# snap-research/GiGL

Measured on AMD Instinct MI355X. Metric: sampled+aggregated edges/s, higher is better.
Workload: dtype f32

## Files before the change

### gigl_amd/csrc/agg.hip

```cpp
#include "wave_reduce.h"
#include "common.h"

#include <cstring>

#include <cstdlib>
#include <type_traits>

#include <hip/hip_fp16.h>

__host__ __device__ static inline float hs_pow2_scale(float m) {
  uint32_t bits;
  memcpy(&bits, &m, 4);
  int e = (int)((bits >> 23) & 0xFF) - 127;
  if (((bits >> 23) & 0xFF) == 0) e = -126;
  int se = 14 - e;
  se = se > 60 ? 60 : (se < -60 ? -60 : se);
  const uint32_t sb = (uint32_t)(se + 127) << 23;
  float s;
  memcpy(&s, &sb, 4);
  return s;
}

namespace {

// ... 1090 lines not shown
        const _Float16 a1 = (_Float16)x;
        fa[s][0][e] = a1;
        fa[s][1][e] = (_Float16)(x - (float)a1);
      }
    if (c + 1 < nc) aload(c + 1);
    if (c + 1 == nc) w2load(0, nc & 1);
    if (c + 1 == nc && wv == 0) {
      short* dst = s_buf[nc & 1] + F2_IMG2;
      if (bias) __builtin_amdgcn_global_load_lds((gptr_t)(reinterpret_cast<const float4_t*>(bias) + lane), (lptr_t)dst, 16, 0, 0);
      else reinterpret_cast<float4_t*>(dst)[lane] = zero4;
    }
    const short* sw = s_buf[c & 1];
#pragma unroll
    for (int s = 0; s < 2; ++s) {
      if (c * 32 + 16 * s >= K) break;
#pragma unroll
      for (int tn = 0; tn < 2; ++tn) {
        half8v_t fw[4][2];
#pragma unroll
        for (int j = 0; j < 4; ++j)
#pragma unroll
          for (int p = 0; p < 2; ++p)
            fw[j][p] = *reinterpret_cast<const half8v_t*>(
                &sw[tn * F2_IMG1 + p * (F2_IMG1 / 2) + split_lds_off(j * 32 + r, 16 * s + 8 * g)]);
        constexpr int HA[3] = {1, 0, 0}, HW[3] = {0, 1, 0};
#pragma unroll
        for (int t = 0; t < 3; ++t)
#pragma unroll
          for (int j = 0; j < 4; ++j)
            acc[4 * tn + j] = __builtin_amdgcn_mfma_f32_32x32x16_f16(fw[j][HW[t]], fa[s][HA[t]], acc[4 * tn + j], 0, 0, 0);
      }
    }
    __syncthreads();
  }
  const float4_t* s_bias = reinterpret_cast<const float4_t*>(s_buf[nc & 1] + F2_IMG2);
  const float s_h = f2_scale[0], o2 = f2_scale[2];
  float16_t acc2[3];
#pragma unroll
  for (int n = 0; n < 3; ++n)
#pragma unroll
    for (int v = 0; v < 16; ++v) acc2[n][v] = 0.f;
#pragma unroll
  for (int rd = 0; rd < 8; ++rd) {
    const _Float16* sw2 = reinterpret_cast<const _Float16*>(s_buf[(nc + rd) & 1]);
    if (rd + 1 < 8) w2load(rd + 1, (nc + rd + 1) & 1);
#pragma unroll
    for (int hf = 0; hf < 2; ++hf) {
      half8v_t h1, h2;
#pragma unroll
      for (int q = 0; q < 2; ++q) {
        const float4_t bq = s_bias[8 * rd + 2 * (2 * hf + q) + g];
#pragma unroll
        for (int t = 0; t < 4; ++t) {
          float x = acc[rd][8 * hf + 4 * q + t] * hs_o + bq[t];
          x = (x > 0.f ? x : 0.f) * s_h;
          const _Float16 a1 = (_Float16)x;
          h1[4 * q + t] = a1;
          h2[4 * q + t] = (_Float16)(x - (float)a1);
        }
      }
#pragma unroll
      for (int n = 0; n < 3; ++n) {
        if (n == 2 && !wr_block) continue;
        const half8v_t w1 = *reinterpret_cast<const half8v_t*>(sw2 + split_lds_off(n * 32 + r, 16 * hf + 8 * g));
        const half8v_t w2 = *reinterpret_cast<const half8v_t*>(sw2 + F2_IMG2 / 2 + split_lds_off(n * 32 + r, 16 * hf + 8 * g));
        acc2[n] = __builtin_amdgcn_mfma_f32_32x32x16_f16(h2, w1, acc2[n], 0, 0, 0);
        acc2[n] = __builtin_amdgcn_mfma_f32_32x32x16_f16(h1, w2, acc2[n], 0, 0, 0);
        acc2[n] = __builtin_amdgcn_mfma_f32_32x32x16_f16(h1, w1, acc2[n], 0, 0, 0);
      }
    }
    if (rd + 1 < 8) __syncthreads();
  }
#pragma unroll
  for (int n = 0; n < 3; ++n) {
    if (n == 2 && !wr_block) continue;
#pragma unroll
    for (int v = 0; v < 16; ++v) {
      const int orow = m0b + wv * 32 + 8 * (v >> 2) + 4 * g + (v & 3);
      if (orow < M) y2[(int64_t)orow * F2_N2 + n * 32 + r] = acc2[n][v] * o2;
    }
  }
}

__global__ __launch_bounds__(256) void fused2_images_kernel(const float* __restrict__ hs, const float* __restrict__ f2,
                                                            const float* __restrict__ w1, int K, const float* __restrict__ w2,
                                                            int n_out, _Float16* __restrict__ w1img,
                                                            _Float16* __restrict__ w2img) {
  const int nc = (K + 31) >> 5;
  const int n1 = 2 * nc * 128 * 32, n2 = 2 * 4 * F2_N2 * 32;
  const int i = blockIdx.x * 256 + threadIdx.x;
  if (i < n1) {
    const int kpos = i & 31, c = (i >> 5) & 127, blk = i >> 12;
    const int tn = blk / nc, ch = blk - tn * nc;
    const int k = 32 * ch + f2_perm(kpos);
    const float x = k < K ? w1[(int64_t)(128 * tn + c) * K + k] * hs[1] : 0.f;
    const _Float16 a1 = (_Float16)x;
    _Float16* img = w1img + (int64_t)blk * F2_IMG1 + split_lds_off(c, kpos);
    img[0] = a1;
    img[F2_IMG1 / 2] = (_Float16)(x - (float)a1);
  } else if (i < n1 + n2) {
    const int e = i - n1;
    const int kpos = e & 31, rest = e >> 5, n = rest % F2_N2, blk = rest / F2_N2;
    const int k = 32 * blk + f2_perm(kpos);
    float x = 0.f;
    if (n < n_out) x = w2[(int64_t)n * 2 * F2_HID + k];
    else if (n >= F2_N2 / 2 && n - F2_N2 / 2 < n_out) x = w2[(int64_t)(n - F2_N2 / 2) * 2 * F2_HID + F2_HID + k];
    x *= f2[1];
    const _Float16 a1 = (_Float16)x;
    _Float16* img = w2img + (int64_t)blk * F2_IMG2 + split_lds_off(n, kpos);
    img[0] = a1;
    img[F2_IMG2 / 2] = (_Float16)(x - (float)a1);
  }
}

__global__ __launch_bounds__(256) void fused2_scale_kernel(const float* __restrict__ hs, const float* __restrict__ b1,
                                                           const float* __restrict__ w2, int n_w2, int K1,
                                                           float* __restrict__ f2) {
  __shared__ float s_m[2][4];
  const int tid = threadIdx.x, gt = blockIdx.x * 256 + tid, stride = gridDim.x * 256;
  float mb = 0.f, mw = 0.f;
  if (b1)
    for (int i = gt; i < F2_HID; i += stride) {
      const float v = fabsf(b1[i]);
      mb = fmaxf(mb, v == v ? v : 0.f);
    }
  for (int i = gt; i < n_w2; i += stride) {
    const float v = fabsf(w2[i]);
    mw = fmaxf(mw, v == v ? v : 0.f);
  }
#pragma unroll
  for (int o = 32; o >= 1; o >>= 1) {
    mb = fmaxf(mb, __shfl_xor(mb, o, 64));
    mw = fmaxf(mw, __shfl_xor(mw, o, 64));
  }
  if ((tid & 63) == 0) {
    s_m[0][tid >> 6] = mb;
    s_m[1][tid >> 6] = mw;
  }
  __syncthreads();
  if (tid == 0) {
    for (int i = 1; i < 4; ++i) {
      mb = fmaxf(mb, s_m[0][i]);
      mw = fmaxf(mw, s_m[1][i]);
    }
    uint32_t* acc = reinterpret_cast<uint32_t*>(f2) + 4;
    atomicMax(acc, __float_as_uint(mb));
    atomicMax(acc + 1, __float_as_uint(mw));
    __threadfence();
    if (atomicAdd(acc + 2, 1u) == gridDim.x - 1) {
      const float b = __uint_as_float(atomicExch(acc, 0u)), w = __uint_as_float(atomicExch(acc + 1, 0u));
      acc[2] = 0u;
      const float inf = __uint_as_float(0x7F800000u);
      float bound = (float)K1 * 1073741824.f * (1.f / hs[0]) * (1.f / hs[1]) + b;
      if (!(bound > 0.f) || !(bound < inf)) bound = 1.f;
      const float s_h = hs_pow2_scale(bound) * 0.5f;
      const float s_w2 = (w > 0.f && w < inf) ? hs_pow2_scale(w) : 1.f;
      f2[0] = s_h;
      f2[1] = s_w2;
      f2[2] = (1.f / s_h) * (1.f / s_w2);
    }
  }
}

__global__ __launch_bounds__(256) void hs_chain_kernel(const float* __restrict__ hs_prev, const float* __restrict__ b_prev,
                                                       int n_b, int k_prev, float fan, const float* __restrict__ w,
                                                       int64_t n_w, float* __restrict__ hs_out) {
  __shared__ float s_m[2][4];
  const int tid = threadIdx.x;
  const int64_t gt = (int64_t)blockIdx.x * 256 + tid, stride = (int64_t)gridDim.x * 256;
  float mb = 0.f, mw = 0.f;
  if (b_prev)
    for (int64_t i = gt; i < n_b; i += stride) {
      const float v = fabsf(b_prev[i]);
      mb = fmaxf(mb, v == v ? v : 0.f);
    }
  const float4* w4 = reinterpret_cast<const float4*>(w);
  const int64_t n4 = ((reinterpret_cast<uintptr_t>(w) & 15) == 0) ? n_w / 4 : 0;
  for (int64_t i = gt; i < n4; i += stride) {
    const float4 v = w4[i];
    const float a = fmaxf(fmaxf(fabsf(v.x), fabsf(v.y)), fmaxf(fabsf(v.z), fabsf(v.w)));
    mw = fmaxf(mw, a == a ? a : 0.f);
  }
  for (int64_t i = n4 * 4 + gt; i < n_w; i += stride) {
    const float v = fabsf(w[i]);
    mw = fmaxf(mw, v == v ? v : 0.f);
  }
#pragma unroll
  for (int o = 32; o >= 1; o >>= 1) {
    mb = fmaxf(mb, __shfl_xor(mb, o, 64));
    mw = fmaxf(mw, __shfl_xor(mw, o, 64));
  }
  if ((tid & 63) == 0) {
    s_m[0][tid >> 6] = mb;
    s_m[1][tid >> 6] = mw;
  }
  __syncthreads();
  if (tid == 0) {
    for (int i = 1; i < 4; ++i) {
      mb = fmaxf(mb, s_m[0][i]);
      mw = fmaxf(mw, s_m[1][i]);
    }
    uint32_t* acc = reinterpret_cast<uint32_t*>(hs_out) + 4;
    atomicMax(acc, __float_as_uint(mb));
    atomicMax(acc + 1, __float_as_uint(mw));
    __threadfence();
    if (atomicAdd(acc + 2, 1u) == gridDim.x - 1) {
      const float b = __uint_as_float(atomicExch(acc, 0u)), wm = __uint_as_float(atomicExch(acc + 1, 0u));
      acc[2] = 0u;
      const float inf = __uint_as_float(0x7F800000u);
      float bound = ((float)k_prev * 1073741824.f * (1.f / hs_prev[0]) * (1.f / hs_prev[1]) + b) * fan;
      if (!(bound > 0.f) || !(bound < inf)) bound = 1.f;
      const float s_h = hs_pow2_scale(bound) * 0.5f;
      const float s_w = (wm > 0.f && wm < inf) ? hs_pow2_scale(wm) : 1.f;
      hs_out[0] = s_h;
      hs_out[1] = s_w;
      hs_out[2] = (1.f / s_h) * (1.f / s_w);
    }
  }
}

template <int OP>
__global__ __launch_bounds__(256) void sage_fused_out_kernel(const float* __restrict__ p, const int32_t* __restrict__ rowptr,
                                                             const int32_t* __restrict__ rowend,
                                                             const int32_t* __restrict__ col,
                                                             const int32_t* __restrict__ root_local, int b, int n_out,
                                                             const float* __restrict__ bias, int act,
                                                             const int32_t* __restrict__ meta, float* __restrict__ out) {
  const int lane = threadIdx.x & 63, sub = lane >> 4, sl = lane & 15;
  const int s = (int)(((int64_t)blockIdx.x * blockDim.x + threadIdx.x) >> 6);
  if (s >= b) return;
  const bool failed = meta[GIGL_META_OVERFLOW] != 0;
  const int i = failed ? -1 : root_local[s];
  float* o = out + (int64_t)s * n_out;
  if (i < 0) {
    const float v = failed ? __builtin_nanf("") : 0.f;
    for (int c = lane; c < n_out; c += 64) o[c] = v;
    return;
  }
  const int e0 = rowptr[i], m = rowend[i] - e0;
  float4_t acc = {0.f, 0.f, 0.f, 0.f};
  if (sl < 12) {
    for (int e = sub; e < m; e += 8) {
// ... 2882 lines not shown

static int32_t linear_tiled_strided(gigl_ctx* ctx, const float* a_tiled, const float* w, const float* bias,
                                    const int32_t* m_dev, int64_t m_cap, int32_t k, int32_t n, int32_t act, float* y,
                                    int32_t ldy, int32_t batch = 1, int64_t a_bstride = 0, int64_t w_bstride = 0,
                                    const float* self_src = nullptr, const uint32_t* self_ids = nullptr,
                                    int32_t d_mean = 0, int32_t self_ld = 0, const float* hs_scale = nullptr, bool self_half = false) {
  const bool hs = hs_scale != nullptr;
  GIGL_REQUIRE(ctx, a_tiled && w && m_dev && y && (k & 3) == 0 && n > 0 && ldy >= n * batch && batch >= 1,
               "bad arguments");
  GIGL_HIP_CHECK(ctx, hipSetDevice(ctx->device));
  if (m_cap == 0) return GIGL_OK;
  hipStream_t st = ctx->stream;
  gigl_prof_scope ps(ctx, GIGL_K_LINEAR);
  const int nkc = (k + 31) / 32;
  const int64_t bm = (m_cap + 127) / 128;
  if (self_src) {
    GIGL_REQUIRE(ctx, batch == 1 && d_mean > 0 && (d_mean & 3) == 0 && d_mean < k && self_ld >= k - d_mean, "bad two-source operand");
    const int nkc_mean = (d_mean + 31) / 32;
    GIGL_REQUIRE(ctx, !self_half || hs, "fp16 self rows go with the half split");
    if (hs && self_half) {
      if (n > 64)
        hipLaunchKernelGGL((linear_split_kernel<2, true, true, false, true, true, true>), dim3((unsigned)(bm * ((n + 127) / 128)), 1u),
                           dim3(256), 0, st, a_tiled, w, bias, m_dev, k, n, act, y, nkc_mean, ldy, (int64_t)0, (int64_t)0,
                           self_src, self_ids, d_mean, self_ld, hs_scale);
      else
        hipLaunchKernelGGL((linear_split_kernel<1, true, true, false, true, true, true>), dim3((unsigned)(bm * ((n + 63) / 64)), 1u),
                           dim3(256), 0, st, a_tiled, w, bias, m_dev, k, n, act, y, nkc_mean, ldy, (int64_t)0, (int64_t)0,
                           self_src, self_ids, d_mean, self_ld, hs_scale);
      GIGL_HIP_CHECK(ctx, hipGetLastError());
      return GIGL_OK;
    }
    if (hs) {
      if (n > 64)
        hipLaunchKernelGGL((linear_split_kernel<2, true, true, false, true, true>), dim3((unsigned)(bm * ((n + 127) / 128)), 1u),
                           dim3(256), 0, st, a_tiled, w, bias, m_dev, k, n, act, y, nkc_mean, ldy, (int64_t)0, (int64_t)0,
                           self_src, self_ids, d_mean, self_ld, hs_scale);
      else
        hipLaunchKernelGGL((linear_split_kernel<1, true, true, false, true, true>), dim3((unsigned)(bm * ((n + 63) / 64)), 1u),
                           dim3(256), 0, st, a_tiled, w, bias, m_dev, k, n, act, y, nkc_mean, ldy, (int64_t)0, (int64_t)0,
                           self_src, self_ids, d_mean, self_ld, hs_scale);
      GIGL_HIP_CHECK(ctx, hipGetLastError());
      return GIGL_OK;
    }
    if (n > 64)
      hipLaunchKernelGGL((linear_split_kernel<2, true, true>), dim3((unsigned)(bm * ((n + 127) / 128)), 1u), dim3(256), 0, st,
                         a_tiled, w, bias, m_dev, k, n, act, y, nkc_mean, ldy, (int64_t)0, (int64_t)0, self_src, self_ids,
                         d_mean, self_ld);
    else
      hipLaunchKernelGGL((linear_split_kernel<1, true, true, false, false, true>), dim3((unsigned)(bm * ((n + 63) / 64)), 1u), dim3(256), 0, st,
                         a_tiled, w, bias, m_dev, k, n, act, y, nkc_mean, ldy, (int64_t)0, (int64_t)0, self_src, self_ids,
                         d_mean, self_ld);
    GIGL_HIP_CHECK(ctx, hipGetLastError());
    return GIGL_OK;
  }
  if (hs) {
    if (n > 64)
      hipLaunchKernelGGL((linear_split_kernel<2, true, false, false, true, true>), dim3((unsigned)(bm * ((n + 127) / 128)), (unsigned)batch),
                         dim3(256), 0, st, a_tiled, w, bias, m_dev, k, n, act, y, nkc, ldy, a_bstride, w_bstride,
                         (const float*)nullptr, (const uint32_t*)nullptr, 0, 0, hs_scale);
    else
      hipLaunchKernelGGL((linear_split_kernel<1, true, false, false, true, true>), dim3((unsigned)(bm * ((n + 63) / 64)), (unsigned)batch),
                         dim3(256), 0, st, a_tiled, w, bias, m_dev, k, n, act, y, nkc, ldy, a_bstride, w_bstride,
                         (const float*)nullptr, (const uint32_t*)nullptr, 0, 0, hs_scale);
    GIGL_HIP_CHECK(ctx, hipGetLastError());
    return GIGL_OK;
  }
  if (n > 64)
    hipLaunchKernelGGL((linear_split_kernel<2, true, false, false, false, true>), dim3((unsigned)(bm * ((n + 127) / 128)), (unsigned)batch), dim3(256), 0,
                       st, a_tiled, w, bias, m_dev, k, n, act, y, nkc, ldy, a_bstride, w_bstride);
  else
    hipLaunchKernelGGL((linear_split_kernel<1, true, false, false, false, true>), dim3((unsigned)(bm * ((n + 63) / 64)), (unsigned)batch), dim3(256), 0,
                       st, a_tiled, w, bias, m_dev, k, n, act, y, nkc, ldy, a_bstride, w_bstride);
  GIGL_HIP_CHECK(ctx, hipGetLastError());
  return GIGL_OK;
}

bool gigl_fused2_shape_ok(int32_t d0, int32_t hid, int32_t n_out) {
  return hid == F2_HID && n_out >= 1 && n_out <= F2_N2 / 2 && (d0 & 3) == 0 && d0 >= 4;
}
static int64_t fused2_img1_bytes(int32_t k1) { return (int64_t)2 * ((k1 + 31) / 32) * F2_IMG1 * 2; }
int64_t gigl_fused2_w2h_bytes(int32_t k1) { return fused2_img1_bytes(k1) + (int64_t)2 * 4 * F2_IMG2 * 2; }
int32_t gigl_fused2_row_floats() { return F2_N2; }

int32_t gigl_fused2_prepare(gigl_ctx* ctx, const float* hs_dev, const float* b1, const float* w1, const float* w2, int32_t n_out,
                            int32_t k1, float* f2, void* w2h) {
  hipLaunchKernelGGL(fused2_scale_kernel, dim3(24), dim3(256), 0, ctx->stream, hs_dev, b1, w2, n_out * 2 * F2_HID, k1, f2);
  _Float16* img1 = reinterpret_cast<_Float16*>(w2h);
  _Float16* img2 = reinterpret_cast<_Float16*>(reinterpret_cast<char*>(w2h) + fused2_img1_bytes(k1));
  const int n = 2 * ((k1 + 31) / 32) * 128 * 32 + 2 * 4 * F2_N2 * 32;
  hipLaunchKernelGGL(fused2_images_kernel, dim3((unsigned)((n + 255) / 256)), dim3(256), 0, ctx->stream, hs_dev,
                     (const float*)f2, w1, k1, w2, n_out, img1, img2);
  GIGL_HIP_CHECK(ctx, hipGetLastError());
  return GIGL_OK;
}

int32_t gigl_hs_chain_update(gigl_ctx* ctx, const float* hs_prev, const float* b_prev, int32_t n_b, int32_t k_prev, float fan,
                             const float* w, int64_t n_w, float* hs_out) {
  int64_t wgs = (n_w / 4 + 255) / 256;
  wgs = wgs < 1 ? 1 : (wgs > 64 ? 64 : wgs);
  hipLaunchKernelGGL(hs_chain_kernel, dim3((unsigned)wgs), dim3(256), 0, ctx->stream, hs_prev, b_prev, n_b, k_prev, fan, w, n_w,
                     hs_out);
  GIGL_HIP_CHECK(ctx, hipGetLastError());
  return GIGL_OK;
}

int32_t gigl_linear_fused2(gigl_ctx* ctx, const float* a_tiled, const float* bias, const int32_t* m_dev, int64_t m_cap,
                           int32_t k, float* y2, const float* self_src, const uint32_t* self_ids, int32_t d_mean,
                           int32_t self_ld, const float* hs_scale, const float* f2, const void* w2h,
                           const int32_t* n_root_rows) {
  GIGL_REQUIRE(ctx, a_tiled && m_dev && y2 && self_src && hs_scale && f2 && w2h && (k & 3) == 0 && d_mean > 0 &&
                        (d_mean & 3) == 0 && d_mean < k && self_ld >= k - d_mean && (((uintptr_t)bias) & 15) == 0,
               "bad arguments");
  GIGL_HIP_CHECK(ctx, hipSetDevice(ctx->device));
  if (m_cap == 0) return GIGL_OK;
  gigl_prof_scope ps(ctx, GIGL_K_LINEAR);
  const _Float16* img1 = reinterpret_cast<const _Float16*>(w2h);
  const _Float16* img2 = reinterpret_cast<const _Float16*>(reinterpret_cast<const char*>(w2h) + fused2_img1_bytes(k));
  hipLaunchKernelGGL(linear_fused2x_kernel, dim3((unsigned)((m_cap + 127) / 128)), dim3(256), 0, ctx->stream, a_tiled, bias,
                     m_dev, k, y2, (d_mean + 31) / 32, self_src, self_ids, d_mean, self_ld, hs_scale, f2, img1, img2,
                     n_root_rows);
  GIGL_HIP_CHECK(ctx, hipGetLastError());
  return GIGL_OK;
}

int32_t gigl_sage_fused_out(gigl_ctx* ctx, const float* p, const int32_t* rowptr, const int32_t* rowend, const int32_t* col,
                            const int32_t* root_local, int32_t b, int32_t n_out, const float* bias, int32_t act,
                            int32_t aggr, const int32_t* meta, float* out) {
  GIGL_REQUIRE(ctx, aggr == GIGL_AGGR_MEAN || aggr == GIGL_AGGR_SUM, "the fused last layer needs a linear reduction");
  if (b == 0) return GIGL_OK;
  gigl_prof_scope ps(ctx, GIGL_K_GATHER_MEAN);
  const dim3 g((unsigned)(((int64_t)b + 3) / 4)), blk(256);
#define GIGL_FOUT(OP)                                                                                                     \
  hipLaunchKernelGGL((sage_fused_out_kernel<OP>), g, blk, 0, ctx->stream, p, rowptr, rowend, col, root_local, b, n_out, bias, \
                     act, meta, out)
  if (aggr == GIGL_AGGR_MEAN) GIGL_FOUT(GIGL_AGGR_MEAN);
  else GIGL_FOUT(GIGL_AGGR_SUM);
#undef GIGL_FOUT
  GIGL_HIP_CHECK(ctx, hipGetLastError());
  return GIGL_OK;
}

int32_t gigl_linear_batched(gigl_ctx* ctx, const float* a, const float* w, const float* bias, const int32_t* m_dev,
                            int64_t m_cap, int32_t k, int32_t n, int32_t act, int32_t batch, int64_t a_bstride,
                            int64_t w_bstride, int32_t ldy, float* y) {
  if (!ctx) return GIGL_E_INVALID_ARG;
  GIGL_REQUIRE(ctx, a && w && m_dev && y, "null argument");
  GIGL_REQUIRE(ctx, k > 0 && (k & 3) == 0 && n > 0 && m_cap >= 0 && batch >= 1 && batch <= 65535 &&
                        (int64_t)ldy >= (int64_t)n * batch && a_bstride >= 0 && w_bstride >= 0,
               "bad sizes (k=%d n=%d batch=%d ldy=%d)", k, n, batch, ldy);
  GIGL_REQUIRE(ctx, act == 0 || act == 1, "bad act %d", act);
  GIGL_HIP_CHECK(ctx, hipSetDevice(ctx->device));
  if (m_cap == 0) return GIGL_OK;
  gigl_prof_scope ps(ctx, GIGL_K_LINEAR);
  const int64_t bm = (m_cap + 127) / 128;
  if (n > 64)
    hipLaunchKernelGGL((linear_split_kernel<2, true>), dim3((unsigned)(bm * ((n + 127) / 128)), (unsigned)batch),
                       dim3(256), 0, ctx->stream, a, w, bias, m_dev, k, n, act, y, 0, ldy, a_bstride, w_bstride);
  else
    hipLaunchKernelGGL((linear_split_kernel<1, true>), dim3((unsigned)(bm * ((n + 63) / 64)), (unsigned)batch),
                       dim3(256), 0, ctx->stream, a, w, bias, m_dev, k, n, act, y, 0, ldy, a_bstride, w_bstride);
  GIGL_HIP_CHECK(ctx, hipGetLastError());
  return GIGL_OK;
}

int32_t gigl_linear_grouped(gigl_ctx* ctx, const gigl_linear_group* groups_dev, int32_t n_groups, int64_t m_cap_max,
                            int32_t k, int32_t n, int32_t act) {
  if (!ctx) return GIGL_E_INVALID_ARG;
  GIGL_REQUIRE(ctx, groups_dev || n_groups == 0, "null argument");
  GIGL_REQUIRE(ctx, k > 0 && (k & 3) == 0 && n > 0 && m_cap_max >= 0 && n_groups >= 0 && n_groups <= 65535,
               "bad sizes (k=%d n=%d groups=%d)", k, n, n_groups);
  GIGL_REQUIRE(ctx, act == 0 || act == 1, "bad act %d", act);
  GIGL_HIP_CHECK(ctx, hipSetDevice(ctx->device));
  if (m_cap_max == 0 || n_groups == 0) return GIGL_OK;
  gigl_prof_scope ps(ctx, GIGL_K_LINEAR);
// ... 446 lines not shown
```

### gigl_amd/csrc/common.h

```cpp
#pragma once

#include <hip/hip_runtime.h>
#include <stdint.h>

#include <cstdarg>
#include <cstdio>
#include <cstdlib>
#include <mutex>
#include <string>
#include <vector>

#include "../../include/gigl_hip.h"

#define GIGL_WAVE 64

struct gigl_ctx {
  int device = 0;
  hipStream_t stream = nullptr;
  bool own_stream = false;
  std::string err;
  char* arena = nullptr;
  int64_t arena_bytes = 0;
  int64_t arena_off = 0;
  uint64_t arena_gen = 0;
  uint32_t prof_mask = 0;
  std::vector<hipEvent_t> prof_ev;
  std::vector<int32_t> prof_id;
  size_t prof_used = 0;
  bool capturing = false;
  double prof_acc_ms[16] = {0};
  int64_t prof_acc_n[16] = {0};
  void* sampler_table = nullptr;
  uint32_t* crc_shift_tbl = nullptr;
  uint32_t* enc_tables = nullptr;
  int32_t enc_tables_d = -1;
  bool wide = false;
};

inline int64_t gigl_level_rows(bool wide, int64_t b, const int32_t* fanouts, int hops, int level_max) {
  int64_t rows = 0, width = b;
  const int top = wide && level_max >= 1 ? hops : level_max;
  for (int i = 0; i <= top; ++i) {
    rows += width;
    if (i < hops) width *= fanouts[i];
  }
  return rows;
}

void gigl_sampler_table_free(gigl_ctx* ctx);

struct gigl_prof_scope {
  gigl_ctx* ctx;
  bool on;
  size_t slot;
  gigl_prof_scope(gigl_ctx* c, int id);
  ~gigl_prof_scope();
};

struct gigl_graph {
  gigl_ctx* ctx = nullptr;
  int64_t n = 0, e = 0;
  int64_t maxdeg = 0;
  bool multi = false;
  int64_t* rowptr = nullptr;
  uint32_t* col = nullptr;
};

struct gigl_feat {
  gigl_ctx* ctx = nullptr;
  int64_t n = 0;
  int32_t d = 0;
  int32_t dtype = 0;
  void* rows = nullptr;
  uint32_t* row_crc = nullptr;
  std::mutex row_crc_mu;
  float absmax = -1.f;
  float absmean_nz = 0.f;
};

int32_t gigl_fail(gigl_ctx* ctx, int32_t code, const char* fmt, ...);

#define GIGL_HIP_CHECK(ctx, expr)                                                          \
  do {                                                                                     \
    hipError_t _e = (expr);                                                                \
    if (_e != hipSuccess)                                                                  \
      return gigl_fail((ctx), _e == hipErrorOutOfMemory ? GIGL_E_OOM : GIGL_E_HIP,         \
                       "%s failed: %s (%s:%d)", #expr, hipGetErrorString(_e), __FILE__,    \
                       __LINE__);                                                          \
  } while (0)

#define GIGL_REQUIRE(ctx, cond, ...)                                  \
  do {                                                                \
    if (!(cond)) return gigl_fail((ctx), GIGL_E_INVALID_ARG, __VA_ARGS__); \
  } while (0)

int32_t gigl_arena_reset(gigl_ctx* ctx, int64_t need_bytes);
void* gigl_arena_alloc(gigl_ctx* ctx, int64_t bytes);

int32_t gigl_lp_rank_metrics_enqueue(gigl_ctx* ctx, hipStream_t st, const float* scores, int64_t ld, int32_t b, int32_t P,
                                     const int32_t* pos_cnt, int32_t n_neg, int32_t neg_col0, const int32_t* neg_valid,
                                     const int32_t* ks, int32_t n_ks, const int32_t* meta_a, const int32_t* meta_b,
                                     double* part, double* acc);
int32_t gigl_graph_compute_maxdeg(gigl_ctx* ctx, gigl_graph* g);
int64_t gigl_linear_weight_grad_chunks(int64_t m_cap, int32_t n, int32_t k, int32_t* rows_per_chunk);
int32_t gigl_linear_weight_grad_sum(gigl_ctx* ctx, const float* part, const float* partb, const int32_t* m_dev, int32_t n, int32_t k,
                                    int32_t rows_per_chunk, float* dw, float* db);
int32_t gigl_linear_weight_grad_parts(gigl_ctx* ctx, const float* dy, const float* a, const float* relu_y, const int32_t* m_dev,
                                      int64_t m_cap, int32_t n, int32_t k, float* part, float* partb);
int32_t gigl_union_build_impl(gigl_ctx* ctx, const uint32_t* roots, const gigl_tree* tree, int32_t group_roots,
                              gigl_union* out, int32_t leaf_global);
void gigl_scan_i64(gigl_ctx* ctx, const int64_t* sizes, int64_t n, int64_t cap, int64_t* out, int32_t* status);
int32_t gigl_gather_reduce_mixed(gigl_ctx* ctx, const void* src, int32_t src_dtype, int32_t d, const uint32_t* gather_ids,
                                 const int32_t* rowptr, const int32_t* rowend, const int32_t* col,
                                 const int32_t* n_rows_dev, int64_t rows_cap, int32_t aggr,
                                 const int32_t* n_local_rows_dev, float* out, int32_t tiled_nkc = 0,
                                 const int32_t* global_map = nullptr, const void* src2 = nullptr,
                                 const void* src3 = nullptr, int32_t no_self = 0, int32_t own_world = 0,
                                 int32_t own_rank = 0, const void* const* peers = nullptr);
int32_t gigl_gather_project_mixed(gigl_ctx* ctx, const float* src_l, const float* src_r, int32_t ld, int32_t d,
                                  const uint32_t* gather_ids, const int32_t* rowptr, const int32_t* rowend,
                                  const int32_t* col, const int32_t* n_rows_dev, int64_t rows_cap, int32_t aggr,
                                  const int32_t* n_local_rows_dev, const float* bias, int32_t act, float* out,
                                  const int32_t* global_map = nullptr, const float* src2 = nullptr,
                                  const float* src3 = nullptr, int32_t ld3 = 0, const int32_t* self_ids = nullptr,
                                  int32_t own_world = 0, int32_t own_rank = 0, const float* const* peers = nullptr);
int32_t gigl_linear_tiled(gigl_ctx* ctx, const float* a_tiled, const float* w, const float* bias, const int32_t* m_dev,
                          int64_t m_cap, int32_t k, int32_t n, int32_t act, float* y, const float* self_src = nullptr,
                          const uint32_t* self_ids = nullptr, int32_t d_mean = 0, int32_t self_ld = 0,
                          const float* hs_scale = nullptr, bool self_half = false);
int32_t gigl_feat_half_split_scale(gigl_ctx* ctx, gigl_feat* feat, float fan, float* s_a);
int32_t gigl_hs_scale_update(gigl_ctx* ctx, const float* w, int64_t n, float s_a, float* hs_dev);
struct gigl_gat_edge_terms {
  const int32_t* eid;
  const float* table;
  int32_t edge_dim;
  const float* att_edge_folded;
  const float* w_edge_msg;
  float* ze;
};
int32_t gigl_gat_input_layer_fused_hs(gigl_ctx* ctx, const void* src, int32_t src_dtype, int32_t d,
                                      const uint32_t* gather_ids, const int32_t* n_local_dev, const float* w,
                                      const float* att_src, const float* att_dst, int32_t heads, int32_t channels,
                                      float negative_slope, const int32_t* rowptr, const int32_t* rowend,
                                      const int32_t* col, const int32_t* n_rows_dev, int64_t rows_cap, const float* bias,
                                      int32_t act, float* scratch, float* out, const float* hs_scale,
                                      const gigl_gat_edge_terms* edge);
int32_t gigl_gat_aggregate_edge_indexed(gigl_ctx* ctx, const float* h, const float* att_src, const float* att_dst,
                                        int32_t heads, int32_t channels, float negative_slope, int32_t concat,
                                        const int32_t* rowptr, const int32_t* rowend, const int32_t* col,
                                        const int32_t* n_nodes_dev, int64_t nodes_cap, const int32_t* n_rows_dev,
                                        int64_t rows_cap, const float* bias, int32_t act, const float* edge_attr,
                                        const int32_t* eid, int32_t edge_dim, int64_t cap_edges,
                                        const float* att_edge_folded, const float* w_edge_msg, float* alpha_scratch,
                                        float* out);
int32_t gigl_gat_input_aggregate_edge(gigl_ctx* ctx, const void* src, int32_t src_dtype, int32_t d, const uint32_t* gather_ids,
                                      const float* u, int32_t heads, float negative_slope, const int32_t* rowptr,
                                      const int32_t* rowend, const int32_t* col, const int32_t* n_rows_dev, int64_t rows_cap,
                                      float* z, const gigl_gat_edge_terms* edge);
int32_t gigl_gat_input_aggregate_backward_edge(gigl_ctx* ctx, const void* src, int32_t src_dtype, int32_t d,
                                               const uint32_t* gather_ids, const float* u, int32_t heads, float negative_slope,
                                               const int32_t* rowptr, const int32_t* rowend, const int32_t* col,
                                               const int32_t* n_rows_dev, int64_t rows_cap, const float* dz, float* du,
                                               const gigl_gat_edge_terms* edge, const float* dze, float* dv);
int32_t gigl_gat_edge_msg_add(gigl_ctx* ctx, const float* ze, const float* w_msg, const float* bias, const int32_t* n_rows_dev,
                              int64_t rows_cap, int32_t heads, int32_t channels, int32_t edge_dim, int32_t act, float* out);
int32_t gigl_gat_edge_msg_backward(gigl_ctx* ctx, const float* dy, int64_t plane, const float* w_msg, const float* z,
                                   const int32_t* n_rows_dev, int64_t rows_cap, int32_t heads, int32_t channels,
                                   int32_t edge_dim, float* dze, float* g_w_msg);
int32_t gigl_gat_aggregate_backward_indexed(gigl_ctx* ctx, const float* h, const float* att_src, const float* att_dst,
                                            int32_t channels, float negative_slope, const int32_t* rowptr,
                                            const int32_t* rowend, const int32_t* col, const int32_t* n_nodes_dev,
                                            int64_t nodes_cap, const int32_t* n_rows_dev, int64_t rows_cap, const float* out_pre,
                                            const float* dout, const float* table, const int32_t* eid, int32_t edge_dim,
                                            const float* att_edge_folded, const float* dze, float* alpha_scratch, float* dh,
                                            float* d_alpha_src, float* d_alpha_dst, float* dv, float* z_out);
int32_t gigl_hs_chain_update(gigl_ctx* ctx, const float* hs_prev, const float* b_prev, int32_t n_b, int32_t k_prev, float fan,
                             const float* w, int64_t n_w, float* hs_out);
bool gigl_fused2_shape_ok(int32_t d0, int32_t hid, int32_t n_out);
int64_t gigl_fused2_w2h_bytes(int32_t k1);
int32_t gigl_fused2_row_floats();
int32_t gigl_fused2_prepare(gigl_ctx* ctx, const float* hs_dev, const float* b1, const float* w1, const float* w2, int32_t n_out,
                            int32_t k1, float* f2, void* w2h);
int32_t gigl_linear_fused2(gigl_ctx* ctx, const float* a_tiled, const float* bias, const int32_t* m_dev, int64_t m_cap,
                           int32_t k, float* y2, const float* self_src, const uint32_t* self_ids, int32_t d_mean,
                           int32_t self_ld, const float* hs_scale, const float* f2, const void* w2h,
                           const int32_t* n_root_rows = nullptr);
int32_t gigl_sage_fused_out(gigl_ctx* ctx, const float* p, const int32_t* rowptr, const int32_t* rowend, const int32_t* col,
                            const int32_t* root_local, int32_t b, int32_t n_out, const float* bias, int32_t act,
                            int32_t aggr, const int32_t* meta, float* out);
bool gigl_half_split_enabled();
int32_t gigl_dev_absmax_f32(gigl_ctx* ctx, const float* p, int64_t n, float* out);
int32_t gigl_feat_absmax(gigl_ctx* ctx, gigl_feat* feat, float* out);

static inline int64_t gigl_align_up(int64_t x, int64_t a) { return (x + a - 1) / a * a; }

static __global__ __launch_bounds__(256) void gigl_fill_u32_kernel(uint32_t* __restrict__ p, uint32_t value, int64_t n_words) {
  for (int64_t i = (int64_t)blockIdx.x * blockDim.x + threadIdx.x; i < n_words; i += (int64_t)gridDim.x * blockDim.x) p[i] = value;
}
static inline void gigl_fill_u32(hipStream_t st, void* p, uint32_t value, int64_t n_words) {
  if (n_words <= 0) return;
  int64_t blocks = (n_words + 255) / 256;
  if (blocks > 2048) blocks = 2048;
  hipLaunchKernelGGL(gigl_fill_u32_kernel, dim3((unsigned)blocks), dim3(256), 0, st, (uint32_t*)p, value, n_words);
}

template <int V>
__global__ __launch_bounds__(256) void gigl_take_rows_kernel(const float* __restrict__ h, const int32_t* __restrict__ root_local,
                                                        int b, int d, const int32_t* __restrict__ meta,
                                                        float* __restrict__ out) {
  const uint32_t dv = (uint32_t)d / V;
  const uint32_t i = blockIdx.x * blockDim.x + threadIdx.x;
  if (i >= (uint32_t)b * dv) return;
  const uint32_t r = i / dv, c = (i - r * dv) * V;
  const bool failed = meta[GIGL_META_OVERFLOW] != 0;
  const int32_t l = failed ? -1 : root_local[r];
  float* dst = out + (int64_t)r * d + c;
  if constexpr (V == 4) {
    float4 v = failed ? make_float4(__builtin_nanf(""), __builtin_nanf(""), __builtin_nanf(""), __builtin_nanf(""))
                      : make_float4(0.f, 0.f, 0.f, 0.f);
    if (l >= 0) v = *reinterpret_cast<const float4*>(h + (int64_t)l * d + c);
    *reinterpret_cast<float4*>(dst) = v;
  } else {
    *dst = failed ? __builtin_nanf("") : (l >= 0 ? h[(int64_t)l * d + c] : 0.f);
  }
}
static inline void gigl_take_rows(hipStream_t st, const float* h, const int32_t* root_local, int b, int d,
                                  const int32_t* meta, float* out) {
  const int64_t total = (int64_t)b * d;
  if ((d & 3) == 0 && (((uintptr_t)out | (uintptr_t)h) & 15) == 0)
    hipLaunchKernelGGL(gigl_take_rows_kernel<4>, dim3((unsigned)((total / 4 + 255) / 256)), dim3(256), 0, st, h, root_local, b,
                       d, meta, out);
  else
    hipLaunchKernelGGL(gigl_take_rows_kernel<1>, dim3((unsigned)((total + 255) / 256)), dim3(256), 0, st, h, root_local, b, d,
                       meta, out);
}

#if defined(__HIPCC__)
__device__ __forceinline__ int gigl_wave_incl_scan(int v) {
  v += __builtin_amdgcn_update_dpp(0, v, 0x111, 0xF, 0xF, true);
  v += __builtin_amdgcn_update_dpp(0, v, 0x112, 0xF, 0xF, true);
  v += __builtin_amdgcn_update_dpp(0, v, 0x114, 0xF, 0xF, true);
  v += __builtin_amdgcn_update_dpp(0, v, 0x118, 0xF, 0xF, true);
  v += __builtin_amdgcn_update_dpp(0, v, 0x142, 0xA, 0xF, false);
  v += __builtin_amdgcn_update_dpp(0, v, 0x143, 0xC, 0xF, false);
  return v;
}

__device__ __forceinline__ float gigl_group_sum(float v, int group) {
#define GIGL_DPP_ADD(CTRL)                                                                                            \
  v += __builtin_bit_cast(float, __builtin_amdgcn_update_dpp(0, __builtin_bit_cast(int, v), CTRL, 0xF, 0xF, true))
  if (group >= 2) GIGL_DPP_ADD(0xB1);
  if (group >= 4) GIGL_DPP_ADD(0x4E);
  if (group >= 8) GIGL_DPP_ADD(0x141);
  if (group >= 16) GIGL_DPP_ADD(0x140);
#undef GIGL_DPP_ADD
  if (group >= 32) {
    const int b = __builtin_bit_cast(int, v);
    const float r0 = __builtin_bit_cast(float, __builtin_amdgcn_readlane(b, 0));
    const float r1 = __builtin_bit_cast(float, __builtin_amdgcn_readlane(b, 16));
    const float r2 = __builtin_bit_cast(float, __builtin_amdgcn_readlane(b, 32));
    const float r3 = __builtin_bit_cast(float, __builtin_amdgcn_readlane(b, 48));
    if (group >= 64) return (r0 + r1) + (r2 + r3);
    return (threadIdx.x & 32) ? r2 + r3 : r0 + r1;
  }
  return v;
// ... 3 lines not shown
```

### gigl_amd/csrc/ctx.hip

```cpp
#include "common.h"

#include <cstring>
#include <new>

int32_t gigl_fail(gigl_ctx* ctx, int32_t code, const char* fmt, ...) {
  char buf[1024];
  va_list ap;
  va_start(ap, fmt);
  vsnprintf(buf, sizeof(buf), fmt, ap);
  va_end(ap);
  if (ctx) ctx->err = buf;
  return code;
}

int32_t gigl_arena_reset(gigl_ctx* ctx, int64_t need_bytes) {
  ctx->arena_off = 0;
  if (need_bytes <= ctx->arena_bytes) return GIGL_OK;
  int64_t want = gigl_align_up(need_bytes + (need_bytes >> 2), 1 << 20);
  if (ctx->arena) {
    GIGL_HIP_CHECK(ctx, hipStreamSynchronize(ctx->stream));
    GIGL_HIP_CHECK(ctx, hipFree(ctx->arena));
    ctx->arena = nullptr;
    ctx->arena_bytes = 0;
  }
// ... 9 lines not shown
  ctx->arena_off = off + bytes;
  return ctx->arena + off;
}

gigl_prof_scope::gigl_prof_scope(gigl_ctx* c, int id) : ctx(c), on(false), slot(0) {
  if (!(c->prof_mask & (1u << id)) || c->prof_used * 2 + 2 > c->prof_ev.size()) return;
  slot = c->prof_used++;
  c->prof_id[slot] = id;
  on = hipEventRecord(c->prof_ev[2 * slot], c->stream) == hipSuccess;
}

gigl_prof_scope::~gigl_prof_scope() {
  if (on) hipEventRecord(ctx->prof_ev[2 * slot + 1], ctx->stream);
}

extern "C" {

int32_t gigl_version(void) { return 100; }

int32_t gigl_profile_enable(gigl_ctx* ctx, uint32_t mask, int32_t capacity) {
  if (!ctx) return GIGL_E_INVALID_ARG;
  GIGL_REQUIRE(ctx, capacity >= 0 && capacity <= (1 << 20), "bad profile capacity");
  GIGL_HIP_CHECK(ctx, hipSetDevice(ctx->device));
  GIGL_HIP_CHECK(ctx, hipStreamSynchronize(ctx->stream));
  ctx->prof_mask = mask;
  ctx->prof_used = 0;
  for (int i = 0; i < 16; ++i) {
    ctx->prof_acc_ms[i] = 0.0;
    ctx->prof_acc_n[i] = 0;
  }
  while (ctx->prof_ev.size() < (size_t)capacity * 2) {
    hipEvent_t e;
    GIGL_HIP_CHECK(ctx, hipEventCreate(&e));
    ctx->prof_ev.push_back(e);
  }
  ctx->prof_id.assign(ctx->prof_ev.size() / 2, -1);
  return GIGL_OK;
}

int32_t gigl_profile_reset(gigl_ctx* ctx) {
  if (!ctx) return GIGL_E_INVALID_ARG;
  GIGL_HIP_CHECK(ctx, hipStreamSynchronize(ctx->stream));
  ctx->prof_used = 0;
  for (int i = 0; i < 16; ++i) {
    ctx->prof_acc_ms[i] = 0.0;
    ctx->prof_acc_n[i] = 0;
  }
  return GIGL_OK;
}

int32_t gigl_profile_read(gigl_ctx* ctx, int32_t kernel_id, double* total_ms, int64_t* launches) {
  if (!ctx) return GIGL_E_INVALID_ARG;
  GIGL_REQUIRE(ctx, kernel_id >= 0 && kernel_id < GIGL_K_COUNT, "bad kernel id");
  GIGL_HIP_CHECK(ctx, hipStreamSynchronize(ctx->stream));
  double tot = ctx->prof_acc_ms[kernel_id];
  int64_t n = ctx->prof_acc_n[kernel_id];
  for (size_t s = 0; s < ctx->prof_used; ++s) {
    if (ctx->prof_id[s] != kernel_id) continue;
    float ms = 0.f;
    GIGL_HIP_CHECK(ctx, hipEventElapsedTime(&ms, ctx->prof_ev[2 * s], ctx->prof_ev[2 * s + 1]));
    tot += ms;
    ++n;
  }
  if (total_ms) *total_ms = tot;
  if (launches) *launches = n;
  return GIGL_OK;
}

int32_t gigl_ctx_create(int32_t device, gigl_ctx** out) {
  if (!out) return GIGL_E_INVALID_ARG;
  *out = nullptr;
  int n = 0;
  if (hipGetDeviceCount(&n) != hipSuccess || n <= 0) return GIGL_E_NO_DEVICE;
  if (device < 0 || device >= n) return GIGL_E_INVALID_ARG;
  gigl_ctx* c = new (std::nothrow) gigl_ctx();
  if (!c) return GIGL_E_OOM;
  c->device = device;
  if (hipSetDevice(device) != hipSuccess ||
      hipStreamCreateWithFlags(&c->stream, hipStreamNonBlocking) != hipSuccess) {
    delete c;
    return GIGL_E_HIP;
  }
  c->own_stream = true;
  *out = c;
  return GIGL_OK;
}

int32_t gigl_ctx_destroy(gigl_ctx* ctx) {
  if (!ctx) return GIGL_OK;
  hipSetDevice(ctx->device);
  if (ctx->stream) hipStreamSynchronize(ctx->stream);
  if (ctx->arena) hipFree(ctx->arena);
  gigl_sampler_table_free(ctx);
  if (ctx->crc_shift_tbl) hipFree(ctx->crc_shift_tbl);
  if (ctx->enc_tables) hipFree(ctx->enc_tables);
  for (hipEvent_t e : ctx->prof_ev) hipEventDestroy(e);
  if (ctx->own_stream && ctx->stream) hipStreamDestroy(ctx->stream);
  delete ctx;
  return GIGL_OK;
}

const char* gigl_last_error(gigl_ctx* ctx) { return ctx ? ctx->err.c_str() : "null ctx"; }

int32_t gigl_ctx_set_wide_workspaces(gigl_ctx* ctx, int32_t on) {
  if (!ctx) return GIGL_E_INVALID_ARG;
  ctx->wide = on != 0;
  return GIGL_OK;
}

int32_t gigl_ctx_set_stream(gigl_ctx* ctx, void* hip_stream) {
  if (!ctx) return GIGL_E_INVALID_ARG;
  if ((hipStream_t)hip_stream == ctx->stream && !ctx->own_stream) return GIGL_OK;
  GIGL_HIP_CHECK(ctx, hipSetDevice(ctx->device));
  GIGL_HIP_CHECK(ctx, hipStreamSynchronize(ctx->stream));
  if (ctx->own_stream && ctx->stream) hipStreamDestroy(ctx->stream);
  ctx->stream = (hipStream_t)hip_stream;
  ctx->own_stream = false;
  return GIGL_OK;
}

int32_t gigl_ctx_synchronize(gigl_ctx* ctx) {
  if (!ctx) return GIGL_E_INVALID_ARG;
  GIGL_HIP_CHECK(ctx, hipStreamSynchronize(ctx->stream));
  return GIGL_OK;
}

int32_t gigl_ctx_reserve(gigl_ctx* ctx, int64_t bytes) {
  if (!ctx) return GIGL_E_INVALID_ARG;
  GIGL_HIP_CHECK(ctx, hipSetDevice(ctx->device));
  return gigl_arena_reset(ctx, bytes);
}

int32_t gigl_memcpy(gigl_ctx* ctx, void* dst, int32_t dst_loc, const void* src, int32_t src_loc,
                    int64_t bytes) {
  if (!ctx) return GIGL_E_INVALID_ARG;
  GIGL_REQUIRE(ctx, bytes >= 0 && (bytes == 0 || (dst && src)), "bad memcpy arguments");
  if (bytes == 0) return GIGL_OK;
  hipMemcpyKind kind = dst_loc == GIGL_LOC_HOST
                           ? (src_loc == GIGL_LOC_HOST ? hipMemcpyHostToHost : hipMemcpyDeviceToHost)
                           : (src_loc == GIGL_LOC_HOST ? hipMemcpyHostToDevice : hipMemcpyDeviceToDevice);
  GIGL_HIP_CHECK(ctx, hipSetDevice(ctx->device));
  GIGL_HIP_CHECK(ctx, hipMemcpyAsync(dst, src, (size_t)bytes, kind, ctx->stream));
  GIGL_HIP_CHECK(ctx, hipStreamSynchronize(ctx->stream));
  return GIGL_OK;
}

static int32_t copy_in(gigl_ctx* ctx, void* dst, const void* src, size_t bytes, int32_t loc) {
  if (bytes == 0) return GIGL_OK;
  GIGL_HIP_CHECK(ctx, hipMemcpyAsync(dst, src, bytes,
                                     loc == GIGL_LOC_HOST ? hipMemcpyHostToDevice
                                                          : hipMemcpyDeviceToDevice,
                                     ctx->stream));
  GIGL_HIP_CHECK(ctx, hipStreamSynchronize(ctx->stream));
  return GIGL_OK;
}

int32_t gigl_graph_load_csc(gigl_ctx* ctx, int64_t n, int64_t e, const int64_t* rowptr,
                            const uint32_t* col, int32_t loc, gigl_graph** out) {
  if (!ctx || !out) return GIGL_E_INVALID_ARG;
  *out = nullptr;
  GIGL_REQUIRE(ctx, n >= 0 && e >= 0 && rowptr && (col || e == 0), "bad CSC arguments");
  GIGL_REQUIRE(ctx, n < (int64_t)GIGL_INVALID, "node ids must fit uint32 (n=%lld)", (long long)n);
  GIGL_REQUIRE(ctx, loc == GIGL_LOC_HOST || loc == GIGL_LOC_DEVICE, "bad loc %d", loc);
  GIGL_HIP_CHECK(ctx, hipSetDevice(ctx->device));
  gigl_graph* g = new (std::nothrow) gigl_graph();
  if (!g) return gigl_fail(ctx, GIGL_E_OOM, "host OOM");
  g->ctx = ctx;
  g->n = n;
  g->e = e;
  hipError_t e1 = hipMalloc((void**)&g->rowptr, (size_t)(n + 1) * sizeof(int64_t));
  hipError_t e2 = e1 == hipSuccess ? hipMalloc((void**)&g->col, (size_t)(e > 0 ? e : 1) * sizeof(uint32_t))
                                   : e1;
  if (e1 != hipSuccess || e2 != hipSuccess) {
    if (g->rowptr) hipFree(g->rowptr);
    delete g;
// ... 92 lines not shown
```

### gigl_amd/csrc/pipeline.hip

```cpp
#include "common.h"
#include "wave_reduce.h"

#include <algorithm>
#include <cmath>
#include <functional>
#include <new>
#include <vector>

namespace {

struct Segment {
  int s0 = 0, s1 = 0;
  hipGraphExec_t exec = nullptr;
};

constexpr int GRAPH_STAGES = 2;

}

struct gigl_sage_plan {
  gigl_ctx* ctx = nullptr;
  gigl_graph* graph = nullptr;
  gigl_feat* feat = nullptr;
  int32_t b = 0, hops = 0;
// ... 129 lines not shown
};

__device__ __forceinline__ void stats_add(unsigned long long* acc, int slot, long long v) {
  for (int off = 32; off > 0; off >>= 1) v += __shfl_xor(v, off, 64);
  if ((threadIdx.x & 63) == 0 && v) atomicAdd(&acc[slot], (unsigned long long)v);
}

__global__ __launch_bounds__(256) void plan_stats_kernel(StatsArgs a, unsigned long long* acc) {
  const int64_t stride = (int64_t)gridDim.x * blockDim.x;
  const int64_t t0 = (int64_t)blockIdx.x * blockDim.x + threadIdx.x;
  const int L = a.hops;
  long long sampled = 0, bytes = 0;
#pragma unroll
  for (int k = 0; k < GIGL_MAX_HOPS; ++k) {
    if (k >= L) break;
    const uint32_t* par = k == 0 ? a.roots : a.nbr[k - 1];
    for (int64_t p = t0; p < a.parents[k]; p += stride) {
      const uint32_t v = par[p];
      if (v == GIGL_INVALID) continue;
      const long long deg = a.g_rowptr[(int64_t)v + 1] - a.g_rowptr[v];
      const long long f = a.fan[k];
      const long long lam = f + (long long)(4.0f * sqrtf((float)f)) + 4;
      bytes += 16 + (deg <= f ? 4 * deg : 8 * (deg < lam ? deg : lam) + 4 * f) + 8 * (deg < f ? deg : f);
      sampled += a.cnt[k][p];
    }
  }
  long long agg[GIGL_MAX_HOPS] = {0, 0, 0, 0};
  const int32_t n_rows = a.meta[GIGL_META_LEVEL0 + L - 1];
  for (int64_t i = t0; i < n_rows && i < a.rows_cap; i += stride) {
    const long long len = a.rowend[i] - a.rowptr[i];
#pragma unroll
    for (int l = 0; l < GIGL_MAX_HOPS; ++l)
      if (l < L && i < a.meta[GIGL_META_LEVEL0 + (L - 1 - l)]) agg[l] += len;
  }
  long long agg_all = 0;
#pragma unroll
  for (int l = 0; l < GIGL_MAX_HOPS; ++l) agg_all += agg[l];
  stats_add(acc, GIGL_STATS_SAMPLED, sampled);
  stats_add(acc, GIGL_STATS_AGGREGATED, agg_all);
  stats_add(acc, GIGL_STATS_EXPAND_BYTES, bytes);
#pragma unroll
  for (int l = 0; l < GIGL_MAX_HOPS; ++l) stats_add(acc, GIGL_STATS_AGG_LAYER0 + l, agg[l]);
  if (t0 == 0) {
    atomicAdd(&acc[GIGL_STATS_UNION_EDGES], (unsigned long long)a.meta[GIGL_META_N_EDGES]);
    atomicAdd(&acc[GIGL_STATS_UNION_NODES], (unsigned long long)a.meta[GIGL_META_N_NODES]);
    atomicAdd(&acc[GIGL_STATS_OVERFLOW], (unsigned long long)a.meta[GIGL_META_OVERFLOW]);
    for (int l = 0; l < L; ++l)
      atomicAdd(&acc[GIGL_STATS_ROWS_LAYER0 + l], (unsigned long long)a.meta[GIGL_META_LEVEL0 + (L - 1 - l)]);
  }
}

int n_stages(const gigl_sage_plan* p) { return 3 + 2 * p->hops; }

bool hs_layers_on() {
  static const bool on = [] {
    const char* e = getenv("GIGL_PLAN_HS_LAYERS");
    return !(e && e[0] == '0');
  }();
  return on;
}

bool fused2_on(const gigl_sage_plan* p) {
  return p->f2_ok && p->kind == 0 && p->hops == 2 && p->tiled && p->two_source && p->hs0 && !p->proj &&
         p->feat->dtype == GIGL_DTYPE_F32 && (p->aggr == GIGL_AGGR_MEAN || p->aggr == GIGL_AGGR_SUM) &&
         (((uintptr_t)p->bias[0]) & 15) == 0;
}

uint32_t stage_kernel_mask(const gigl_sage_plan* p, int s) {
  if (s == 0) return (1u << GIGL_K_EXPAND) | (1u << GIGL_K_EXPAND_HEAVY) | (1u << GIGL_K_FIND_HEAVY);
  if (s == 1)
    return (1u << GIGL_K_UNION_INSERT) | (1u << GIGL_K_UNION_RELAX) | (1u << GIGL_K_UNION_NODES) |
           (1u << GIGL_K_UNION_EDGE_SORT) | (1u << GIGL_K_UNION_CSR);
  if (s == n_stages(p) - 1) return 0;
  return ((s - 2) & 1) ? (1u << GIGL_K_LINEAR) : (1u << GIGL_K_GATHER_MEAN);
}

int32_t enqueue_stage(gigl_sage_plan* p, int s, const uint32_t* roots, int32_t sampling_seed, int32_t mode,
                      float* out) {
  gigl_ctx* ctx = p->ctx;
  const int L = p->hops;
  if (s == 0)
    return gigl_sample_khop(ctx, p->graph, roots, p->b, p->fanouts, p->hops, sampling_seed, mode, &p->tree);
  if (s == 1) {
    int32_t rc = gigl_union_build_impl(ctx, roots, &p->tree, p->group_roots, &p->un,
                                       p->leaf_global ? (1 | (p->graph->multi ? 2 : 0)) : 0);
    if (rc != GIGL_OK) return rc;
    hipLaunchKernelGGL(guard_levels_kernel, dim3(1), dim3(64), 0, ctx->stream, p->un.meta, p->hops,
                       (int32_t)(p->act_rows < 0x7FFFFFFF ? p->act_rows : 0x7FFFFFFF));
    GIGL_HIP_CHECK(ctx, hipGetLastError());
    if (p->efeat) {
      const int64_t rows_cap = gigl_level_rows(p->wide, p->b, p->fanouts, L, L - 1);
      int64_t blocks = (rows_cap + 3) / 4;
      if (blocks > 256 * 16) blocks = 256 * 16;
      const int32_t* n_local = p->leaf_global ? (L >= 2 ? p->un.meta + GIGL_META_LEVEL0 + (L - 2) : p->zero_dev) : nullptr;
      hipLaunchKernelGGL(plan_edge_ids_kernel, dim3((unsigned)blocks), dim3(256), 0, ctx->stream, p->graph->rowptr, p->graph->col,
                         p->graph->n, p->un.nodes, p->un.rowptr, p->un.rowend, p->un.col, p->un.meta + GIGL_META_LEVEL0 + (L - 1),
                         n_local, rows_cap, p->un.cap_edges + (p->alias_rows ? p->last_slots : 0), p->eid);
      GIGL_HIP_CHECK(ctx, hipGetLastError());
    }
    return GIGL_OK;
  }
  if (s == n_stages(p) - 1) {
    const int dout = p->dims[L];
    if (fused2_on(p)) {
      const int32_t rc = gigl_sage_fused_out(ctx, p->hbuf[0], p->un.rowptr, p->un.rowend, p->un.col, p->un.root_local, p->b,
                                             dout, p->bias[L - 1], p->act_last ? 1 : 0, p->aggr, p->un.meta, out);
      if (rc != GIGL_OK) return rc;
    } else {
      gigl_take_rows(ctx->stream, p->hbuf[(L - 1) & 1], p->un.root_local, p->b, dout, p->un.meta, out);
    }
    if (p->l2_normalize)
      hipLaunchKernelGGL(l2_normalize_rows_kernel, dim3((unsigned)((p->b + 3) / 4)), dim3(256), 0, ctx->stream, out, p->b, dout);
    GIGL_HIP_CHECK(ctx, hipGetLastError());
    return GIGL_OK;
  }
  const int l = (s - 2) >> 1;
  if (l == 1 && fused2_on(p)) return GIGL_OK;
  const int32_t* n_rows = p->un.meta + GIGL_META_LEVEL0 + (L - 1 - l);
  const int d = p->dims[l];
  const int64_t rows_cap = gigl_level_rows(p->wide, p->b, p->fanouts, L, L - 1 - l);
  int64_t width = p->b;
  for (int i = 0; i <= L - 1 - l; ++i) width *= p->fanouts[i];
  if (p->wide) width = 0;
  if (p->kind == 1) {
    const int act = (l < L - 1 || p->act_last) ? 1 : 0;
    const bool first = ((s - 2) & 1) == 0;
    if (l == 0) {
      if (!first) return GIGL_OK;
      const int32_t* n_local = p->leaf_global ? (L >= 2 ? p->un.meta + GIGL_META_LEVEL0 + (L - 2) : p->zero_dev) : nullptr;
      if (p->hs0) {
        const int32_t rc = gigl_hs_scale_update(ctx, p->w[0], (int64_t)p->heads[0] * p->channels[0] * d, p->hs_sa, p->hs_dev);
        if (rc != GIGL_OK) return rc;
      }
      gigl_gat_edge_terms et{};
      if (p->efeat) {
        et.eid = p->eid;
        et.table = (const float*)p->efeat->rows;
        et.edge_dim = p->efeat->d;
        et.att_edge_folded = p->att_edge[0];
        et.w_edge_msg = p->w_msg[0];
        et.ze = p->ze;
      }
      return gigl_gat_input_layer_fused_hs(ctx, p->feat->rows, p->feat->dtype, d, p->un.nodes, n_local, p->w[0], p->att_src[0],
                                           p->att_dst[0], p->heads[0], p->channels[0], p->slope, p->un.rowptr, p->un.rowend,
                                           p->un.col, n_rows, rows_cap, p->bias[0], act, p->gat_scratch, p->hbuf[0],
                                           p->hs0 ? p->hs_dev : nullptr, p->efeat ? &et : nullptr);
    }
    const int32_t* n_src = p->un.meta + GIGL_META_LEVEL0 + (L - l);
    int64_t src_cap = rows_cap + width;
    if (first)
      return gigl_linear(ctx, p->hbuf[(l - 1) & 1], p->w[l], nullptr, n_src, src_cap, d, p->dims[l + 1], 0, p->hw);
    if (p->efeat)
      return gigl_gat_aggregate_edge_indexed(ctx, p->hw, p->att_src[l], p->att_dst[l], p->heads[l], p->channels[l], p->slope, 1,
                                             p->un.rowptr, p->un.rowend, p->un.col, n_src, src_cap, n_rows, rows_cap, p->bias[l],
                                             act, (const float*)p->efeat->rows, p->eid, p->efeat->d,
                                             p->un.cap_edges + (p->alias_rows ? p->last_slots : 0), p->att_edge[l], p->w_msg[l],
                                             p->alpha_scratch, p->hbuf[l & 1]);
    return gigl_gat_aggregate(ctx, p->hw, p->att_src[l], p->att_dst[l], p->heads[l], p->channels[l], p->slope, 1,
                              p->un.rowptr, p->un.rowend, p->un.col, n_src, src_cap, n_rows, rows_cap, p->bias[l], act,
                              p->alpha_scratch, p->hbuf[l & 1]);
  }
  if (l == 0 && p->proj) {
    if (((s - 2) & 1) != 0) return GIGL_OK;
    const int act = (l < L - 1 || p->act_last) ? 1 : 0;
    return gigl_gather_project_mixed(
        ctx, p->proj, p->proj + p->dims[1], 2 * p->dims[1], p->dims[1], p->un.nodes, p->un.rowptr, p->un.rowend, p->un.col, n_rows, rows_cap,
        p->aggr, p->leaf_global ? (L >= 2 ? p->un.meta + GIGL_META_LEVEL0 + (L - 2) : p->zero_dev) : nullptr, p->bias[0],
        act, p->hbuf[0]);
  }
  const bool self_half = l == 0 && p->hs0 && p->feat->dtype == GIGL_DTYPE_F16;
  const bool two_src = p->tiled && p->two_source && (l > 0 || p->feat->dtype == GIGL_DTYPE_F32 || self_half);
  const int32_t nkc = p->tiled ? ((two_src ? d : 2 * d) + 31) / 32 : 0;
  if (((s - 2) & 1) == 0) {
    if (p->tiled) {
      if (l == 0)
        return gigl_gather_reduce_mixed(
            ctx, p->feat->rows, p->feat->dtype, d, p->un.nodes, p->un.rowptr, p->un.rowend, p->un.col, n_rows, rows_cap,
            p->aggr, p->leaf_global ? (L >= 2 ? p->un.meta + GIGL_META_LEVEL0 + (L - 2) : p->zero_dev) : nullptr,
            p->abuf, nkc, nullptr, nullptr, nullptr, two_src ? 1 : 0);
      return gigl_gather_reduce_mixed(ctx, p->hbuf[(l - 1) & 1], GIGL_DTYPE_F32, d, nullptr, p->un.rowptr, p->un.rowend,
                                      p->un.col, n_rows, rows_cap, p->aggr, nullptr, p->abuf, nkc, nullptr, nullptr, nullptr,
                                      two_src ? 1 : 0);
    }
    if (l == 0 && p->leaf_global)
      return gigl_gather_reduce_mixed(ctx, p->feat->rows, p->feat->dtype, d, p->un.nodes, p->un.rowptr, p->un.rowend,
                                      p->un.col, n_rows, rows_cap, p->aggr,
                                      L >= 2 ? p->un.meta + GIGL_META_LEVEL0 + (L - 2) : p->zero_dev, p->abuf);
    if (l == 0)
      return gigl_gather_reduce(ctx, p->feat->rows, p->feat->dtype, d, p->un.nodes, p->un.rowptr, p->un.rowend,
                                p->un.col, n_rows, rows_cap, p->aggr, p->abuf);
    return gigl_gather_reduce(ctx, p->hbuf[(l - 1) & 1], GIGL_DTYPE_F32, d, nullptr, p->un.rowptr, p->un.rowend,
                              p->un.col, n_rows, rows_cap, p->aggr, p->abuf);
  }
  const int act = (l < L - 1 || p->act_last) ? 1 : 0;
  const float* hs_scale = nullptr;
  if (l == 0 && p->hs0 && p->tiled) {
    const int32_t rc = gigl_hs_scale_update(ctx, p->w[0], (int64_t)p->dims[1] * 2 * d, p->hs_sa, p->hs_dev);
    if (rc != GIGL_OK) return rc;
    hs_scale = p->hs_dev;
  }
  if (l >= 1 && two_src && p->hs0 && !p->proj && p->hs_layer[l] && hs_layers_on()) {
    const float* prev = l == 1 ? p->hs_dev : p->hs_layer[l - 1];
    float fan = 1.f;
    if (p->aggr == GIGL_AGGR_SUM)
      for (int k = 0; k < p->hops; ++k) fan = (float)p->fanouts[k] > fan ? (float)p->fanouts[k] : fan;
    int32_t rc = gigl_hs_chain_update(ctx, prev, p->bias[l - 1], p->dims[l], 2 * p->dims[l - 1], fan, p->w[l],
                                      (int64_t)p->dims[l + 1] * 2 * d, p->hs_layer[l]);
    if (rc != GIGL_OK) return rc;
    return gigl_linear_tiled(ctx, p->abuf, p->w[l], p->bias[l], n_rows, rows_cap, 2 * d, p->dims[l + 1], act,
                             p->hbuf[l & 1], p->hbuf[(l - 1) & 1], nullptr, d, d, p->hs_layer[l]);
  }
  if (l == 0 && fused2_on(p)) {
    int32_t rc = gigl_fused2_prepare(ctx, p->hs_dev, p->bias[0], p->w[0], p->w[1], p->dims[2], 2 * d, p->f2_dev, p->w2h);
    if (rc != GIGL_OK) return rc;
    return gigl_linear_fused2(ctx, p->abuf, p->bias[0], n_rows, rows_cap, 2 * d, p->hbuf[0], (const float*)p->feat->rows,
                              p->un.nodes, d, d, hs_scale, p->f2_dev, p->w2h,
                              getenv("GIGL_F2_ALL_WR") ? nullptr : p->un.meta + GIGL_META_LEVEL0);
  }
  if (two_src)
    return gigl_linear_tiled(ctx, p->abuf, p->w[l], p->bias[l], n_rows, rows_cap, 2 * d, p->dims[l + 1], act,
                             p->hbuf[l & 1], l == 0 ? (const float*)p->feat->rows : p->hbuf[(l - 1) & 1],
                             l == 0 ? p->un.nodes : nullptr, d, d, hs_scale, self_half);
  if (p->tiled)
    return gigl_linear_tiled(ctx, p->abuf, p->w[l], p->bias[l], n_rows, rows_cap, 2 * d, p->dims[l + 1], act,
                             p->hbuf[l & 1], nullptr, nullptr, 0, 0, hs_scale);
  return gigl_linear(ctx, p->abuf, p->w[l], p->bias[l], n_rows, rows_cap, 2 * d, p->dims[l + 1], act,
                     p->hbuf[l & 1]);
}

int32_t enqueue_range(gigl_sage_plan* p, int s0, int s1, const uint32_t* roots, int32_t sampling_seed, int32_t mode,
                      float* out) {
  for (int s = s0; s < s1; ++s) {
    int32_t rc = enqueue_stage(p, s, roots, sampling_seed, mode, out);
    if (rc != GIGL_OK) return rc;
  }
  return GIGL_OK;
}

void drop_graphs(gigl_sage_plan* p) {
  for (Segment& sg : p->segs)
    if (sg.exec) hipGraphExecDestroy(sg.exec);
  p->segs.clear();
  p->captured = false;
}

int32_t capture_segments(gigl_sage_plan* p, int32_t sampling_seed, int32_t mode) {
  gigl_ctx* ctx = p->ctx;
  const int n = n_stages(p);
  const uint32_t mask = ctx->prof_mask;
  int s = 0;
  while (s < n) {
    Segment sg;
    sg.s0 = s;
    const bool timed = (stage_kernel_mask(p, s) & mask) != 0 || s == n - 1;
    int e = s + 1;
    while (e < n - 1 && ((stage_kernel_mask(p, e) & mask) != 0) == timed && s != n - 1 && !(p->split && e == GRAPH_STAGES)) ++e;
    sg.s1 = e;
    if (!timed) {
      hipGraph_t graph = nullptr;
      hipStream_t keep = ctx->stream;
      if (p->split && sg.s1 <= GRAPH_STAGES) ctx->stream = p->gstream;
      hipError_t err = hipStreamBeginCapture(ctx->stream, hipStreamCaptureModeThreadLocal);
      int32_t rc = GIGL_OK;
      if (err == hipSuccess) {
        rc = enqueue_range(p, sg.s0, sg.s1, p->roots_buf, sampling_seed, mode, p->out_buf);
        hipError_t e2 = hipStreamEndCapture(ctx->stream, &graph);
        if (rc == GIGL_OK && e2 != hipSuccess) err = e2;
      }
      ctx->stream = keep;
      if (rc == GIGL_OK && err == hipSuccess) err = hipGraphInstantiate(&sg.exec, graph, nullptr, nullptr, 0);
      if (graph) hipGraphDestroy(graph);
      if (rc != GIGL_OK) return rc;
      if (err != hipSuccess) {
        sg.exec = nullptr;
        return gigl_fail(ctx, GIGL_E_HIP, "capturing stages [%d,%d) of the batch pipeline failed: %s", sg.s0, sg.s1,
                         hipGetErrorString(err));
      }
    }
    p->segs.push_back(sg);
    s = e;
  }
  return GIGL_OK;
}



__device__ __forceinline__ void ce_root_row(const float* __restrict__ out, int width, const int32_t* __restrict__ root_local,
                                            const int64_t* __restrict__ labels, const int32_t* __restrict__ n_valid_dev, int b,
                                            const int32_t* __restrict__ meta, float* __restrict__ dout,
                                            float* __restrict__ loss_rows) {
  const int lane = threadIdx.x & 63;
  const int i = (blockIdx.x * blockDim.x + threadIdx.x) >> 6;
  if (i >= b) return;
  const int n_valid = *n_valid_dev;
  const int32_t rl = root_local[i];
  if (i >= n_valid || rl < 0 || meta[GIGL_META_OVERFLOW] != 0) {
    if (lane == 0) loss_rows[i] = meta[GIGL_META_OVERFLOW] != 0 ? __builtin_nanf("") : 0.f;
    return;
  }
  const float* row = out + (int64_t)rl * width;
  float mx = -3.402823466e38f;
// ... 2864 lines not shown
```

### gigl_amd/csrc/sample.hip

```cpp
#include "common.h"

#include <cstdlib>
#include <mutex>
#include <type_traits>

namespace {

constexpr uint64_t P1 = 0x9E3779B185EBCA87ULL;
constexpr uint64_t P2 = 0xC2B2AE3D27D4EB4FULL;
constexpr uint64_t P3 = 0x165667B19E3779F9ULL;
constexpr uint64_t P5 = 0x27D4EB2F165667C5ULL;
constexpr uint64_t SPARK_SEED = 42ULL;
constexpr uint64_t SIGN = 0x8000000000000000ULL;

__device__ __forceinline__ uint64_t xxh64_i32_ordered(uint32_t x) {
  uint64_t h = (SPARK_SEED + P5 + 4ULL) ^ ((uint64_t)x * P1);
  h = ((h << 23) | (h >> 41)) * P2 + P3;
  h ^= h >> 33;
  h *= P2;
  h ^= h >> 29;
  h *= P3;
  h ^= h >> 32;
  return h ^ SIGN;
}
// ... 334 lines not shown
  __device__ __forceinline__ bool filter_positions(const uint32_t* flat, uint32_t n, uint32_t T, uint32_t base,
                                                   uint32_t* lk, uint32_t* li) {
    const bool all = T == 0xFFFFFFFFu;
    uint32_t count = 0;
    const uint32_t nchunks = (n + 63u) >> 6;
    const uint32_t* src = flat + base;
    for (uint32_t c = 0; c < nchunks; c += 4) {
      uint32_t kk[4];
#pragma unroll
      for (uint32_t t = 0; t < 4; ++t) {
        const uint32_t i = (c + t) * 64u + (uint32_t)lane + 1u;
        kk[t] = 0xFFFFFFFFu;
        if constexpr (SRC == SRC_FLAT) {
          if (c + t < nchunks) kk[t] = src[i];
        } else {
          kk[t] = (uint32_t)(xxh64_i32_ordered(i + base) >> 32);
        }
      }
#pragma unroll
      for (uint32_t t = 0; t < 4; ++t) {
        if (c + t >= nchunks) break;
        const uint32_t i = (c + t) * 64u + (uint32_t)lane + 1u;
        const uint32_t k = kk[t] & dmask;
        offer(k, i, i <= n && (all || k < T), count, lk, li);
      }
    }
    return finish(count, lk, li);
  }
  __device__ __forceinline__ bool filter_level(const uint2* ent, uint32_t cnt, uint32_t n, uint32_t T, uint32_t base,
                                               uint32_t* lk, uint32_t* li) {
    uint32_t count = 0;
    for (uint32_t e0 = 0; e0 < cnt; e0 += 128u) {
      const uint32_t ea = e0 + (uint32_t)lane, eb = ea + 64u;
      uint2 xa = make_uint2(0u, 0xFFFFFFFFu), xb = xa;
      if (ea < cnt) xa = ent[ea];
      if (eb < cnt) xb = ent[eb];
      const uint32_t ia = xa.x - base, ib = xb.x - base;
      offer(xa.y & dmask, ia, (uint32_t)(ia - 1u) < n && xa.y < T, count, lk, li);
      if (e0 + 64u < cnt) offer(xb.y & dmask, ib, (uint32_t)(ib - 1u) < n && xb.y < T, count, lk, li);
    }
    return finish(count, lk, li);
  }
  __device__ __forceinline__ void serial(const RangeTable& tb, uint32_t n, uint32_t base, uint32_t T, bool in_table) {
    reset_best();
    if (!in_table) {
      scan_row(nullptr, (int64_t)n, base);
      return;
    }
    const uint32_t T4 = T >= (1u << 30) ? 0xFFFFFFFFu : 4u * T;
    const int l4 = T4 == 0xFFFFFFFFu ? 0 : min((int)__builtin_clz(T4 - 1u), tb.levels);
    if (l4 > 0) {
      if (scan_level(tb, l4, T4, n, base)) return;
      reset_best();
    }
    if constexpr (FAST) {
      scan_row(tb.flat, (int64_t)n, base);
      if (readlane32(idx, f - 1) == 0xFFFFFFFFu) tie = true;
    } else {
      scan_row(nullptr, (int64_t)n, base);
    }
  }
};

enum { ROW_INVALID = 0, ROW_COPY = 1, ROW_FLAT = 2, ROW_LEVEL = 3, ROW_HASH = 4, ROW_SERIAL = 5, ROW_SERIAL_HASH = 6,
       ROW_SKIP = 7 };

struct __attribute__((aligned(32))) RowDesc {
  int64_t s;
  uint32_t n;
  uint32_t base;
  uint32_t T;
  uint32_t kind_cnt;
  const void* ptr;
};

__device__ __forceinline__ float filter_lambda(int f) { return (float)f + 4.f * __builtin_sqrtf((float)f) + 4.f; }

constexpr int WORK_LISTS = 64;
constexpr int WORK_CNT_STRIDE = 32;

struct WorkLists {
  uint32_t* items;
  int32_t* count;
  int64_t cap;
  int32_t iters;
  int32_t wgs;
};

__host__ __device__ static inline int64_t work_list_cap(int64_t n_parents) {
  return ((n_parents / 256 + 1 + WORK_LISTS - 1) / WORK_LISTS) * 256;
}
static inline int64_t expand_desc_bytes(int64_t n_parents) {
  return (n_parents + 1) * (int64_t)sizeof(RowDesc) + WORK_LISTS * work_list_cap(n_parents) * 4 +
         WORK_LISTS * WORK_CNT_STRIDE * 4 + 512;
}

__global__ void work_counts_zero_kernel(int32_t* count) { count[threadIdx.x * WORK_CNT_STRIDE] = 0; }

__global__ __launch_bounds__(256) void plan_rows_kernel(ExpandArgs a, RangeTable tb, RowDesc* __restrict__ desc,
                                                        int64_t* heavy_list, int32_t* heavy_count, WorkLists wl) {
  __shared__ int32_t s_wave[4];
  __shared__ int32_t s_base;
  const uint32_t p = blockIdx.x * 256u + threadIdx.x;
  const int lane = threadIdx.x & 63, w = threadIdx.x >> 6;
  bool real = false;
  if (p <= (uint32_t)a.n_parents) {
    RowDesc d{};
    if (p == (uint32_t)a.n_parents) {
      d.kind_cnt = ROW_SKIP;
      desc[p] = d;
    } else {
      uint32_t v, ksum;
      parent_of(a, p, v, ksum);
      uint32_t* out = a.out_nbr + (int64_t)p * a.f;
      if (v == GIGL_INVALID || (int64_t)v >= a.n_nodes) {
        for (int j = 0; j < a.f; ++j) out[j] = GIGL_INVALID;
        a.out_cnt[p] = 0;
      } else {
        int64_t deg;
        if (a.peer_world) {
          const uint32_t q = v / a.peer_world, rk = v - q * a.peer_world;
          const int64_t* rp = a.peer_rowptr[rk];
          const int64_t s0 = rp[q];
          deg = rp[q + 1] - s0;
          d.s = ((int64_t)rk << 48) | s0;
        } else {
          d.s = a.rowptr[v];
          deg = a.rowptr[v + 1] - d.s;
        }
        d.n = (uint32_t)deg;
        d.base = ksum + (uint32_t)a.hash_add;
        if (deg <= a.f && !a.multi) {
          const uint32_t* row = row_of_desc(a, d.s);
          for (int j = 0; j < a.f; ++j) out[j] = j < (int)deg ? row[j] : GIGL_INVALID;
          a.out_cnt[p] = (int32_t)deg;
        } else if (deg <= a.f) {
          d.kind_cnt = ROW_COPY;
          desc[p] = d;
          real = true;
        } else {
          const bool in_table = (uint64_t)d.base + (uint64_t)deg < tb.dom;
          const float lam = filter_lambda(a.f);
          d.T = d.n <= 64u ? 0xFFFFFFFFu
                           : (uint32_t)fminf(lam * 4294967296.f * __builtin_amdgcn_rcpf((float)d.n), 4294967040.f);
          uint32_t kind;
          if (!in_table) {
            if (deg > HEAVY_DEG) {
              kind = ROW_SKIP;
              if (heavy_list) heavy_list[atomicAdd(heavy_count, 1)] = (int64_t)p;
            } else {
              kind = lam <= 56.f ? ROW_HASH : ROW_SERIAL_HASH;
            }
          } else if (lam > 56.f) {
            kind = ROW_SERIAL;
          } else {
            const int l = min((int)__builtin_clz(d.T - 1u), tb.levels);
            if (l == 0 || d.n <= (uint32_t)a.flat_max) {
              kind = ROW_FLAT;
              d.ptr = tb.flat;
            } else {
              const int gs = TBL_IDX_SHIFT + l;
              const uint32_t* off = tb.off[l];
              const uint32_t start = off[(d.base + 1u) >> gs], end = off[((d.base + d.n) >> gs) + 1u];
              if (end - start > 256u) {
                kind = ROW_SERIAL;
              } else {
                kind = ROW_LEVEL | ((end - start) << 3);
                d.ptr = tb.lvl[l] + start;
              }
            }
          }
          d.kind_cnt = kind;
          desc[p] = d;
          real = (kind & 7u) != ROW_SKIP;
        }
      }
    }
  }
  const unsigned long long m = __ballot(real);
  if (lane == 0) s_wave[w] = (int32_t)__popcll(m);
  __syncthreads();
  const int list = (int)(blockIdx.x % WORK_LISTS);
  if (threadIdx.x == 0) {
    const int32_t tot = s_wave[0] + s_wave[1] + s_wave[2] + s_wave[3];
    s_base = tot ? atomicAdd(&wl.count[list * WORK_CNT_STRIDE], tot) : 0;
  }
  __syncthreads();
// ... 509 lines not shown
  own = new TableOwner();
  own->device = dev;
  uint64_t dom = want_dom + want_dom / 4;
  if (dom > DOM_CAP) dom = DOM_CAP;
  dom = dom / S0 * S0;
  if (dom < S0) dom = S0;
  const int L = TBL_MAX_LEVELS;
  const uint32_t n_tiles = (uint32_t)(dom >> TBL_TILE_SHIFT);
  auto up = [](size_t x) { return (x + 255) & ~(size_t)255; };
  size_t off_elems[TBL_MAX_LEVELS + 1] = {0}, off_at[TBL_MAX_LEVELS + 1] = {0};
  size_t bytes = up((size_t)dom * 4);
  for (int l = 1; l <= L; ++l) {
    const int gs = TBL_IDX_SHIFT + l;
    off_elems[l] = (size_t)((dom + (1ull << gs) - 1) >> gs) + 1;
    off_at[l] = bytes;
    bytes = up(bytes + off_elems[l] * 4);
  }
  const size_t cnt_at = bytes;
  bytes = up(bytes + (size_t)L * n_tiles * 4);
  const size_t total_at = bytes;
  bytes += 256;
  auto fail_build = [&](int32_t code, const char* what, hipError_t e) {
    if (own->mem) hipFree(own->mem);
    if (own->mem2) hipFree(own->mem2);
    delete own;
    return gigl_fail(ctx, code, "%s (hash threshold table over %llu j): %s", what, (unsigned long long)dom,
                     hipGetErrorString(e));
  };
  hipError_t e = hipMalloc(&own->mem, bytes);
  if (e != hipSuccess) {
    own->mem = nullptr;
    return fail_build(GIGL_E_OOM, "hipMalloc failed", e);
  }
  char* m0 = (char*)own->mem;
  uint32_t* flat = (uint32_t*)m0;
  uint32_t* cnt = (uint32_t*)(m0 + cnt_at);
  uint32_t* total = (uint32_t*)(m0 + total_at);
  hipLaunchKernelGGL(table_flat_kernel, dim3((unsigned)((dom + 255) / 256)), dim3(256), 0, ctx->stream, flat, dom);
  hipLaunchKernelGGL(table_count_kernel, dim3(n_tiles), dim3(256), 0, ctx->stream, flat, cnt, n_tiles, L);
  hipLaunchKernelGGL(table_scan_kernel, dim3((unsigned)L), dim3(1024), 0, ctx->stream, cnt, n_tiles, total);
  uint32_t h_total[TBL_MAX_LEVELS + 1] = {0};
  e = hipGetLastError();
  if (e == hipSuccess) e = hipMemcpyAsync(h_total, total, sizeof(h_total), hipMemcpyDeviceToHost, ctx->stream);
  if (e == hipSuccess) e = hipStreamSynchronize(ctx->stream);
  if (e != hipSuccess) return fail_build(GIGL_E_HIP, "counting failed", e);
  size_t lvl_at[TBL_MAX_LEVELS + 1] = {0}, bytes2 = 0;
  for (int l = 1; l <= L; ++l) {
    lvl_at[l] = bytes2;
    bytes2 = up(bytes2 + (size_t)h_total[l] * 8 + 8);
  }
  e = hipMalloc(&own->mem2, bytes2);
  if (e != hipSuccess) {
    own->mem2 = nullptr;
    return fail_build(GIGL_E_OOM, "hipMalloc of the level lists failed", e);
  }
  RangeTable t{};
  t.dom = dom;
  t.levels = L;
  t.flat = flat;
  TableBuild tbuild{};
  tbuild.flat = flat;
  tbuild.tile_off = cnt;
  tbuild.total = total;
  tbuild.n_tiles = n_tiles;
  tbuild.levels = L;
  tbuild.dom = dom;
  for (int l = 1; l <= L; ++l) {
    tbuild.lvl[l] = (uint2*)((char*)own->mem2 + lvl_at[l]);
    tbuild.off[l] = (uint32_t*)(m0 + off_at[l]);
    t.lvl[l] = tbuild.lvl[l];
    t.off[l] = tbuild.off[l];
  }
  hipLaunchKernelGGL(table_fill_kernel, dim3(n_tiles), dim3(256), 0, ctx->stream, tbuild);
  e = hipGetLastError();
  if (e == hipSuccess) e = hipStreamSynchronize(ctx->stream);
  if (e != hipSuccess) return fail_build(GIGL_E_HIP, "filling failed", e);
  own->t = t;
  own->refs = 1;
  g_device_table[dev] = own;
  ctx->sampler_table = own;
  return GIGL_OK;
}

int32_t run_expand(gigl_ctx* ctx, const ExpandArgs& a_in, const RangeTable& tb, bool covered,
                   int64_t* heavy_list, int32_t* heavy_count, RowDesc* desc) {
  ExpandArgs a = a_in;
  if (a.f > GIGL_FAST_FANOUT) {
    gigl_prof_scope ps(ctx, GIGL_K_EXPAND);
    int64_t wgs = a.n_parents < 8192 ? a.n_parents : 8192;
    hipLaunchKernelGGL(expand_wide_kernel, dim3((unsigned)wgs), dim3(256), 0, ctx->stream, a);
    GIGL_HIP_CHECK(ctx, hipGetLastError());
    return GIGL_OK;
  }
  a.proxy_drop = 0;
  if (const char* e = getenv("GIGL_SAMPLER_PROXY_BITS")) {
    int bits = atoi(e);
    if (bits >= 1 && bits <= 32) a.proxy_drop = 32 - bits;
  }
  static const int32_t flat_max = [] {
    const char* e = getenv("GIGL_EXPAND_FLAT_MAX");
    return e ? atoi(e) : 128;
  }();
  a.flat_max = flat_max;
  if (!covered) gigl_fill_u32(ctx->stream, heavy_count, 0u, 1);
  WorkLists wl{};
  wl.cap = work_list_cap(a.n_parents);
  wl.items = reinterpret_cast<uint32_t*>(desc + a.n_parents + 1);
  wl.count = reinterpret_cast<int32_t*>(wl.items + (int64_t)WORK_LISTS * wl.cap);
  wl.count = reinterpret_cast<int32_t*>(((uintptr_t)wl.count + 127) & ~(uintptr_t)127);
  hipLaunchKernelGGL(work_counts_zero_kernel, dim3(1), dim3(WORK_LISTS), 0, ctx->stream, wl.count);
  {
    gigl_prof_scope ps(ctx, GIGL_K_EXPAND);
    hipLaunchKernelGGL(plan_rows_kernel, dim3((unsigned)(a.n_parents / 256 + 1)), dim3(256), 0, ctx->stream, a, tb,
                       desc, covered ? nullptr : heavy_list, heavy_count, wl);
    int64_t wgs = ((a.n_parents + 7) / 8 + 15) / 16 * 16;
    static const int64_t wgs_max = [] {
      const char* e = getenv("GIGL_EXPAND_WGS");
      const int64_t v = e ? atoll(e) : 2048;
      return v < 16 ? (int64_t)16 : v / 16 * 16;
    }();
    if (wgs > wgs_max) wgs = wgs_max;
    static const int32_t iters = [] {
      const char* e = getenv("GIGL_EXPAND_ITERS");
      const int v = e ? atoi(e) : 16;
      return v < 0 ? 0 : v;
    }();
    wl.iters = iters;
    wl.wgs = (int32_t)wgs;
    if (iters > 0) {
      const int64_t stride = wgs * 4 / WORK_LISTS;
      const int64_t steps = (wl.cap / 2 + stride - 1) / stride;
      wgs *= (steps + iters - 1) / iters;
    }
    hipLaunchKernelGGL(expand_rows_kernel, dim3((unsigned)wgs), dim3(256), 0, ctx->stream, a, tb, (const RowDesc*)desc, wl);
  }
  if (!covered) {
    gigl_prof_scope ps(ctx, GIGL_K_EXPAND_HEAVY);
    int64_t hb = a.n_parents < 2048 ? a.n_parents : 2048;
    hipLaunchKernelGGL(expand_heavy_kernel, dim3((unsigned)hb), dim3(256), 0, ctx->stream, a, heavy_list,
                       heavy_count);
  }
  GIGL_HIP_CHECK(ctx, hipGetLastError());
  return GIGL_OK;
}

uint64_t window_bound(const gigl_graph* g, int32_t hops, int32_t first_counter, int32_t sampling_seed) {
  uint64_t worst = 0;
  for (int k = 0; k < hops; ++k) {
    int64_t add = (int64_t)sampling_seed * (int64_t)(first_counter + k);
    if (add < 0 || add > (int64_t)0x7FFFFFFF) return ~0ULL;
    uint64_t hi = (uint64_t)(k + 1) * (uint64_t)(g->n > 0 ? g->n - 1 : 0) + (uint64_t)add + (uint64_t)g->maxdeg;
    if (hi > worst) worst = hi;
  }
  return worst;
}

__device__ __forceinline__ uint32_t mix32(uint32_t x) {
  x ^= x >> 16;
  x *= 0x7feb352dU;
  x ^= x >> 15;
  x *= 0x846ca68bU;
  x ^= x >> 16;
  return x;
}

__global__ __launch_bounds__(256) void expand_fast_kernel(ExpandArgs a) {
  const int lane = threadIdx.x & 63;
  const int wave_in_block = threadIdx.x >> 6;
  const int64_t waves_total = (int64_t)gridDim.x * 4;
  for (int64_t p = (int64_t)blockIdx.x * 4 + wave_in_block; p < a.n_parents; p += waves_total) {
    uint32_t v, ksum;
    parent_of(a, p, v, ksum);
    uint32_t* out = a.out_nbr + p * a.f;
    const int f = a.f;
    if (v == GIGL_INVALID || (int64_t)v >= a.n_nodes) {
      if (lane < f) out[lane] = GIGL_INVALID;
      if (lane == 0) a.out_cnt[p] = 0;
      continue;
    }
    const int64_t s = a.rowptr[v];
    const int64_t deg = a.rowptr[v + 1] - s;
    const uint32_t* row = a.col + s;
    if (deg <= f) {
      if (lane < f) out[lane] = lane < deg ? row[lane] : GIGL_INVALID;
      if (lane == 0) a.out_cnt[p] = (int32_t)deg;
      continue;
    }
    if (lane < f) {
      int64_t lo = (int64_t)lane * deg / f, hi = (int64_t)(lane + 1) * deg / f;
      uint32_t r = mix32(mix32(ksum + (uint32_t)a.hash_add) ^ (uint32_t)(lane * 0x9E3779B9u));
      int64_t pos = lo + (int64_t)(((uint64_t)r * (uint64_t)(hi - lo)) >> 32);
      out[lane] = row[pos];
    }
// ... 50 lines not shown
int32_t gigl_sample_khop(gigl_ctx* ctx, gigl_graph* g, const uint32_t* roots, int32_t b,
                         const int32_t* fanouts, int32_t hops, int32_t sampling_seed, int32_t mode,
                         gigl_tree* out) {
  if (!ctx) return GIGL_E_INVALID_ARG;
  GIGL_REQUIRE(ctx, g && (roots || b == 0) && fanouts && out, "null argument");
  GIGL_REQUIRE(ctx, hops >= 1 && hops <= GIGL_MAX_HOPS, "hops must be in [1,%d]", GIGL_MAX_HOPS);
  GIGL_REQUIRE(ctx, b >= 0, "negative batch");
  GIGL_REQUIRE(ctx, mode == GIGL_MODE_SPARK_HASH || mode == GIGL_MODE_FAST || mode == GIGL_MODE_REPLACE,
               "bad mode %d", mode);
  int64_t parents = b;
  for (int k = 0; k < hops; ++k) {
    if (fanouts[k] < 1 || fanouts[k] > GIGL_MAX_FANOUT)
      return gigl_fail(ctx, GIGL_E_UNSUPPORTED, "fanout[%d]=%d outside [1,%d]", k, fanouts[k],
                       GIGL_MAX_FANOUT);
    if (mode != GIGL_MODE_SPARK_HASH && fanouts[k] > GIGL_FAST_FANOUT)
      return gigl_fail(ctx, GIGL_E_UNSUPPORTED, "fanout[%d]=%d: the non-parity modes take fanouts up to %d", k, fanouts[k],
                       GIGL_FAST_FANOUT);
    GIGL_REQUIRE(ctx, out->nbr[k] && out->cnt[k], "tree buffers for hop %d are null", k);
    parents *= fanouts[k];
    GIGL_REQUIRE(ctx, parents < (int64_t)1 << 31, "tree too large");
  }
  GIGL_HIP_CHECK(ctx, hipSetDevice(ctx->device));
  out->hops = hops;
  out->b = b;
  for (int k = 0; k < hops; ++k) out->fanouts[k] = fanouts[k];
  if (b == 0) return GIGL_OK;

  RangeTable tb{};
  bool covered = false;
  int32_t rc = GIGL_OK;
  if (mode == GIGL_MODE_SPARK_HASH) {
    const uint64_t bound = window_bound(g, hops, 1, sampling_seed);
    const uint64_t cap = table_cap_j();
    rc = ensure_table(ctx, bound == ~0ULL ? (1ull << 20) : (bound + 1 < cap ? bound + 1 : cap));
    if (rc != GIGL_OK) return rc;
    tb = ((TableOwner*)ctx->sampler_table)->t;
    covered = bound != ~0ULL && bound < tb.dom;
  }

  int64_t* heavy_list = nullptr;
  int32_t* heavy_count = nullptr;
  RowDesc* desc = nullptr;
  if (mode == GIGL_MODE_SPARK_HASH) {
    int64_t max_parents = b, q = b;
    for (int k = 0; k + 1 < hops; ++k) {
      q *= fanouts[k];
      if (q > max_parents) max_parents = q;
    }
    rc = gigl_arena_reset(ctx, expand_desc_bytes(max_parents) + max_parents * 8 + 1024);
    if (rc != GIGL_OK) return rc;
    desc = (RowDesc*)gigl_arena_alloc(ctx, expand_desc_bytes(max_parents));
    if (!covered) {
      heavy_list = (int64_t*)gigl_arena_alloc(ctx, max_parents * 8);
      heavy_count = (int32_t*)gigl_arena_alloc(ctx, 256);
    }
    if (!desc || (!covered && (!heavy_list || !heavy_count))) return gigl_fail(ctx, GIGL_E_OOM, "arena exhausted");
  }

  ExpandArgs a{};
  a.rowptr = g->rowptr;
  a.col = g->col;
  a.n_nodes = g->n;
  a.multi = g->multi ? 1 : 0;
  a.roots = roots;
  parents = b;
  for (int k = 0; k < hops; ++k) {
    a.hop = k;
    a.n_parents = parents;
    a.f = fanouts[k];
    a.fan[k] = fanouts[k];
    a.hash_add = (int32_t)((uint32_t)sampling_seed * (uint32_t)(k + 1));
    a.out_nbr = out->nbr[k];
    a.out_cnt = out->cnt[k];
    if (mode == GIGL_MODE_FAST || mode == GIGL_MODE_REPLACE) {
      int64_t blocks = (parents + 3) / 4;
      if (blocks > 256 * 32) blocks = 256 * 32;
      gigl_prof_scope ps(ctx, GIGL_K_EXPAND);
      if (mode == GIGL_MODE_FAST)
        hipLaunchKernelGGL(expand_fast_kernel, dim3((unsigned)blocks), dim3(256), 0, ctx->stream, a);
      else
        hipLaunchKernelGGL(expand_replace_kernel, dim3((unsigned)blocks), dim3(256), 0, ctx->stream, a);
      GIGL_HIP_CHECK(ctx, hipGetLastError());
    } else {
      rc = run_expand(ctx, a, tb, covered, heavy_list, heavy_count, desc);
      if (rc != GIGL_OK) return rc;
    }
    a.anc[k] = out->nbr[k];
    parents *= fanouts[k];
  }
  return GIGL_OK;
}

int32_t gigl_sample_khop_peer(gigl_ctx* ctx, const int64_t* const* peer_rowptr, const uint32_t* const* peer_col,
                              int32_t world, int64_t n_global, int64_t max_window_end, const uint32_t* roots, int32_t b,
                              const int32_t* fanouts, int32_t hops, int32_t sampling_seed, gigl_tree* out) {
  if (!ctx) return GIGL_E_INVALID_ARG;
  GIGL_REQUIRE(ctx, peer_rowptr && peer_col && (roots || b == 0) && fanouts && out, "null argument");
  GIGL_REQUIRE(ctx, hops >= 1 && hops <= GIGL_MAX_HOPS && b >= 0 && world >= 1 && world < (1 << 15), "bad shape");
  int64_t parents = b, max_parents = b;
  for (int k = 0; k < hops; ++k) {
    if (fanouts[k] < 1 || fanouts[k] > GIGL_FAST_FANOUT)
      return gigl_fail(ctx, GIGL_E_UNSUPPORTED, "peer-mapped sampling takes fan-outs up to %d (fanout[%d]=%d)", GIGL_FAST_FANOUT, k,
                       fanouts[k]);
    GIGL_REQUIRE(ctx, out->nbr[k] && out->cnt[k], "tree buffers for hop %d are null", k);
    if (parents > max_parents) max_parents = parents;
    parents *= fanouts[k];
    GIGL_REQUIRE(ctx, parents < (int64_t)1 << 31, "tree too large");
  }
  GIGL_HIP_CHECK(ctx, hipSetDevice(ctx->device));
  out->hops = hops;
  out->b = b;
  for (int k = 0; k < hops; ++k) out->fanouts[k] = fanouts[k];
  if (b == 0) return GIGL_OK;
  const uint64_t cap = table_cap_j();
  if (max_window_end < 0 || (uint64_t)max_window_end + 1 > cap)
    return gigl_fail(ctx, GIGL_E_UNSUPPORTED, "peer-mapped sampling needs a window bound inside the threshold table (max_window_end)");
  int32_t rc = ensure_table(ctx, (uint64_t)max_window_end + 1);
  if (rc != GIGL_OK) return rc;
  const RangeTable tb = ((TableOwner*)ctx->sampler_table)->t;
  if ((uint64_t)max_window_end >= tb.dom)
    return gigl_fail(ctx, GIGL_E_UNSUPPORTED, "peer-mapped sampling: the window bound exceeds the threshold table");
  rc = gigl_arena_reset(ctx, expand_desc_bytes(max_parents) + 1024);
  if (rc != GIGL_OK) return rc;
  RowDesc* desc = (RowDesc*)gigl_arena_alloc(ctx, expand_desc_bytes(max_parents));
  if (!desc) return gigl_fail(ctx, GIGL_E_OOM, "arena exhausted");
  ExpandArgs a{};
  a.peer_rowptr = peer_rowptr;
  a.peer_col = peer_col;
  a.peer_world = (uint32_t)world;
  a.n_nodes = n_global;
  a.multi = 0;
  a.roots = roots;
  parents = b;
  for (int k = 0; k < hops; ++k) {
    a.hop = k;
    a.n_parents = parents;
    a.f = fanouts[k];
    a.fan[k] = fanouts[k];
    a.hash_add = (int32_t)((uint32_t)sampling_seed * (uint32_t)(k + 1));
    a.out_nbr = out->nbr[k];
    a.out_cnt = out->cnt[k];
    rc = run_expand(ctx, a, tb, true, nullptr, nullptr, desc);
    if (rc != GIGL_OK) return rc;
    a.anc[k] = out->nbr[k];
    parents *= fanouts[k];
  }
  return GIGL_OK;
}

int32_t gigl_expand_frontier(gigl_ctx* ctx, gigl_graph* shard, const uint32_t* nodes, const uint32_t* ksums,
                             int64_t m, int32_t f, int32_t hash_add, int32_t world, int64_t max_window_end,
                             uint32_t* out_nbr, int32_t* out_cnt) {
  if (!ctx) return GIGL_E_INVALID_ARG;
  GIGL_REQUIRE(ctx, shard && (m == 0 || (nodes && ksums && out_nbr && out_cnt)), "null argument");
  GIGL_REQUIRE(ctx, world >= 1 && m >= 0 && m < ((int64_t)1 << 31), "bad sizes");
  if (f < 1 || f > GIGL_MAX_FANOUT)
    return gigl_fail(ctx, GIGL_E_UNSUPPORTED, "fanout %d outside [1,%d]", f, GIGL_MAX_FANOUT);
  GIGL_HIP_CHECK(ctx, hipSetDevice(ctx->device));
  if (m == 0) return GIGL_OK;
  const uint64_t cap = table_cap_j();
  const bool bounded = max_window_end >= 0;
  const uint64_t bound = bounded ? (uint64_t)max_window_end : ~0ULL;
  int32_t rc = ensure_table(ctx, !bounded ? (1ull << 20) : (bound + 1 < cap ? bound + 1 : cap));
  if (rc != GIGL_OK) return rc;
  const RangeTable tb = ((TableOwner*)ctx->sampler_table)->t;
  const bool covered = bounded && bound < tb.dom;
  int64_t* heavy_list = nullptr;
  int32_t* heavy_count = nullptr;
  rc = gigl_arena_reset(ctx, expand_desc_bytes(m) + m * 8 + 1024);
  if (rc != GIGL_OK) return rc;
  RowDesc* desc = (RowDesc*)gigl_arena_alloc(ctx, expand_desc_bytes(m));
  if (!covered) {
    heavy_list = (int64_t*)gigl_arena_alloc(ctx, m * 8);
    heavy_count = (int32_t*)gigl_arena_alloc(ctx, 256);
  }
  if (!desc || (!covered && (!heavy_list || !heavy_count))) return gigl_fail(ctx, GIGL_E_OOM, "arena exhausted");
  ExpandArgs a{};
  a.rowptr = shard->rowptr;
  a.col = shard->col;
  a.n_nodes = shard->n;
  a.multi = shard->multi ? 1 : 0;
  a.hop = 0;
  a.n_parents = m;
  a.f = f;
  a.fan[0] = f;
  a.hash_add = hash_add;
  a.out_nbr = out_nbr;
  a.out_cnt = out_cnt;
  a.ex_nodes = nodes;
  a.ex_ksum = ksums;
  a.row_div = (uint32_t)world;
  return run_expand(ctx, a, tb, covered, heavy_list, heavy_count, desc);
}

int32_t gigl_sample_positives(gigl_ctx* ctx, gigl_graph* g_out, const uint32_t* roots, int32_t b,
                              int32_t f, int32_t sampling_seed, int32_t mode, uint32_t* pos,
                              int32_t* cnt) {
  return gigl_sample_out_neighbors(ctx, g_out, roots, b, f, sampling_seed, 3, mode, pos, cnt);
}

int32_t gigl_sample_out_neighbors(gigl_ctx* ctx, gigl_graph* g_out, const uint32_t* roots, int32_t b,
                                  int32_t f, int32_t sampling_seed, int32_t counter, int32_t mode, uint32_t* pos,
                                  int32_t* cnt) {
  if (!ctx) return GIGL_E_INVALID_ARG;
  GIGL_REQUIRE(ctx, counter >= 1 && counter <= 64, "permutation call counter %d outside [1,64]", counter);
  GIGL_REQUIRE(ctx, g_out && (roots || b == 0) && pos && cnt, "null argument");
  GIGL_REQUIRE(ctx, mode == GIGL_MODE_SPARK_HASH, "positives are parity-mode only");
  if (f < 1 || f > GIGL_MAX_FANOUT)
    return gigl_fail(ctx, GIGL_E_UNSUPPORTED, "num positives %d outside [1,%d]", f, GIGL_MAX_FANOUT);
  GIGL_HIP_CHECK(ctx, hipSetDevice(ctx->device));
  if (b == 0) return GIGL_OK;
  int32_t rc = gigl_arena_reset(ctx, expand_desc_bytes(b) + (int64_t)(b + 1) * 8 + 1024);
  if (rc != GIGL_OK) return rc;
  RowDesc* desc = (RowDesc*)gigl_arena_alloc(ctx, expand_desc_bytes(b));
  int64_t* heavy_list = (int64_t*)gigl_arena_alloc(ctx, (int64_t)b * 8);
  int32_t* heavy_count = (int32_t*)gigl_arena_alloc(ctx, 256);
  if (!desc || !heavy_list || !heavy_count) return gigl_fail(ctx, GIGL_E_OOM, "arena exhausted");
  ExpandArgs a{};
  a.rowptr = g_out->rowptr;
  a.col = g_out->col;
  a.n_nodes = g_out->n;
  a.multi = g_out->multi ? 1 : 0;
  a.roots = roots;
  a.hop = 0;
  a.n_parents = b;
  a.f = f;
  a.fan[0] = f;
  a.hash_add = (int32_t)((uint32_t)sampling_seed * (uint32_t)counter);
  a.out_nbr = pos;
  a.out_cnt = cnt;
  const uint64_t bound = window_bound(g_out, 1, counter, sampling_seed);
  const uint64_t cap = table_cap_j();
  rc = ensure_table(ctx, bound == ~0ULL ? (1ull << 20) : (bound + 1 < cap ? bound + 1 : cap));
  if (rc != GIGL_OK) return rc;
  const RangeTable tb = ((TableOwner*)ctx->sampler_table)->t;
  return run_expand(ctx, a, tb, bound != ~0ULL && bound < tb.dom, heavy_list, heavy_count, desc);
}

}
```

### gigl_amd/csrc/union.hip

```cpp
#include "common.h"

#include <mutex>

#include <cstdlib>

static hipError_t lds_opt_in(int device, int site, const void* fn, int bytes, const void* fn2 = nullptr, int bytes2 = 0) {
  static std::mutex mu;
  static uint32_t done[256] = {0};
  std::lock_guard<std::mutex> lk(mu);
  const uint32_t bit = 1u << site;
  uint32_t& d = done[device & 255];
  if (d & bit) return hipSuccess;
  hipError_t e = hipFuncSetAttribute(fn, hipFuncAttributeMaxDynamicSharedMemorySize, bytes);
  if (e == hipSuccess && fn2) e = hipFuncSetAttribute(fn2, hipFuncAttributeMaxDynamicSharedMemorySize, bytes2);
  if (e == hipSuccess) d |= bit;
  return e;
}

static bool lg_big_cap_wide() {
  static const bool wide = [] {
    const char* e = getenv("GIGL_LG_BIG_CAP");
    return !(e && atoi(e) > 0 && atoi(e) <= 4096);
  }();
  return wide;
// ... 1174 lines not shown
  const int lane = threadIdx.x & 63, w = threadIdx.x >> 6;
  const int32_t nq = *sort_count;
  const int32_t wave = (blockIdx.x * blockDim.x + threadIdx.x) >> 6;
  const int32_t waves_total = (gridDim.x * blockDim.x) >> 6;
  int32_t edges = 0;
  for (int32_t q = wave; q < nq; q += waves_total) {
    const int32_t i = sort_rows[q];
    const int32_t s = rowptr[i], m = rowend[i] - s;
    if (m > MED_ROW) {
      if (lane == 0) big_rows[atomicAdd(big_count, 1)] = i;
      continue;
    }
    if (m <= 64) {
      const int32_t v = lane < m ? col[s + lane] : 0x7FFFFFFF;
      bool firstv = lane < m;
      for (int j = 0; j < m; ++j) {
        const int32_t vj = __builtin_amdgcn_readlane(v, j);
        if (j < lane && vj == v) firstv = false;
      }
      const unsigned long long fm = __ballot(firstv);
      int32_t pos = 0;
      for (int j = 0; j < m; ++j) {
        const int32_t vj = __builtin_amdgcn_readlane(v, j);
        pos += ((fm >> j) & 1ull) && vj < v ? 1 : 0;
      }
      if (firstv) col[s + pos] = v;
      const int32_t len = (int32_t)__popcll(fm);
      if (lane == 0) rowend[i] = s + len;
      edges += len;
      continue;
    }
    int32_t* H = s_h[w];
    int32_t* U = s_u[w];
#pragma unroll
    for (int r = 0; r < MED_HASH / 64; ++r) H[lane + 64 * r] = -1;
    wave_lds_sync();
    for (int r = 0; r * 64 < m; ++r) {
      const int idx = lane + 64 * r;
      if (idx < m) {
        const int32_t v = col[s + idx];
        uint32_t h = hash_u32((uint32_t)v) & (MED_HASH - 1);
        for (;;) {
          const int32_t prev = atomicCAS(&H[h], -1, v);
          if (prev == -1 || prev == v) break;
          h = (h + 1) & (MED_HASH - 1);
        }
      }
    }
    wave_lds_sync();
    int32_t u = 0;
#pragma unroll
    for (int r = 0; r < MED_HASH / 64; ++r) {
      const int32_t v = H[lane + 64 * r];
      const unsigned long long vm = __ballot(v != -1);
      if (v != -1) U[u + (int32_t)__popcll(vm & ((1ull << lane) - 1ull))] = v;
      u += (int32_t)__popcll(vm);
    }
    wave_lds_sync();
    int32_t mine[MED_ROW / 64], pos[MED_ROW / 64];
#pragma unroll
    for (int r = 0; r < MED_ROW / 64; ++r) {
      mine[r] = lane + 64 * r < u ? U[lane + 64 * r] : 0x7FFFFFFF;
      pos[r] = 0;
    }
    for (int j = 0; j < u; ++j) {
      const int32_t x = U[j];
#pragma unroll
      for (int r = 0; r < MED_ROW / 64; ++r) pos[r] += x < mine[r] ? 1 : 0;
    }
#pragma unroll
    for (int r = 0; r < MED_ROW / 64; ++r)
      if (lane + 64 * r < u) col[s + pos[r]] = mine[r];
    if (lane == 0) rowend[i] = s + u;
    edges += u;
    wave_lds_sync();
  }
  if (lane == 0 && edges) atomicAdd(&edge_counters[(blockIdx.x & 31) * ec_stride], edges);
}

template <int CAP>
__global__ __launch_bounds__(1024) void lg2_row_sort_big_kernel(const int32_t* rowptr, int32_t* rowend, int32_t* col,
                                                                const int32_t* big_rows, const int32_t* big_count,
                                                                int32_t* overflow, int32_t* edge_counters,
                                                                int32_t* ticket, int32_t* meta, int ec_stride = 1,
                                                                const int32_t* tile_edges = nullptr, int32_t n_tile_edges = 0) {
  extern __shared__ int32_t lds[];
  int32_t* A = lds;
  int32_t* B = lds + CAP;
  __shared__ int32_t s_cnt[NBUCKET];
  __shared__ int32_t s_off[NBUCKET + 1];
  __shared__ int32_t s_w[16];
  __shared__ int32_t s_sub[16][64];
  __shared__ int32_t s_min, s_max, s_uniq, s_last;
  const int tid = threadIdx.x, lane = tid & 63, w = tid >> 6;
  const int32_t nb = *big_count;
  constexpr uint32_t HMASK = 2 * CAP - 1;
  int32_t edges = 0;
  for (int32_t r = blockIdx.x; r < nb; r += gridDim.x) {
    const int32_t i = big_rows[r];
    const int32_t s = rowptr[i], m_raw = rowend[i] - s;
    for (int q = tid; q < 2 * CAP; q += 1024) lds[q] = -1;
    if (tid == 0) s_uniq = 0;
    __syncthreads();
    for (int q = tid; q < m_raw; q += 1024) {
      if (*(volatile int32_t*)&s_uniq > CAP) break;
      const int32_t v = col[s + q];
      uint32_t h = hash_u32((uint32_t)v) & HMASK;
      for (uint32_t probes = 0; probes <= HMASK; ++probes) {
        const int32_t prev = atomicCAS(&lds[h], -1, v);
        if (prev == -1) {
          atomicAdd(&s_uniq, 1);
          break;
        }
        if (prev == v) break;
        h = (h + 1) & HMASK;
      }
    }
    __syncthreads();
    const int32_t m = s_uniq;
    __syncthreads();
    if (m > CAP) {
      const int32_t md = huge_row_sort_distinct(col + s, m_raw, lds, s_w, 2 * CAP);
      if (tid == 0) {
        rowend[i] = s + md;
        edges += md;
      }
      __syncthreads();
      continue;
    }
    if (tid == 0) s_uniq = 0;
    __syncthreads();
    for (int q = tid; q < 2 * CAP; q += 1024) {
      const int32_t v = lds[q];
      if (v != -1) col[s + atomicAdd(&s_uniq, 1)] = v;
    }
    __syncthreads();
    if (tid == 0) {
      rowend[i] = s + m;
      edges += m;
      s_min = 0x7FFFFFFF;
      s_max = 0;
    }
    s_cnt[tid] = 0;
    __syncthreads();
    if (m <= 1) continue;
    int32_t mn = 0x7FFFFFFF, mx = 0;
    for (int q = tid; q < m; q += 1024) {
      const int32_t v = col[s + q];
      A[q] = v;
      mn = min(mn, v);
      mx = max(mx, v);
    }
    for (int off = 32; off > 0; off >>= 1) {
      mn = min(mn, __shfl_xor(mn, off, 64));
      mx = max(mx, __shfl_xor(mx, off, 64));
    }
    if (lane == 0) {
      atomicMin(&s_min, mn);
      atomicMax(&s_max, mx);
    }
    __syncthreads();
    const int64_t vmin = s_min, span = (int64_t)s_max - s_min + 1;
    for (int q = tid; q < m; q += 1024) atomicAdd(&s_cnt[(int)(((int64_t)(A[q] - vmin) * NBUCKET) / span)], 1);
    __syncthreads();
    {
      const int32_t v = s_cnt[tid];
      int32_t incl = v;
      for (int off = 1; off < 64; off <<= 1) {
// ... 11 lines not shown
    __syncthreads();
    for (int q = tid; q < m; q += 1024) {
      const int32_t v = A[q];
      B[atomicAdd(&s_cnt[(int)(((int64_t)(v - vmin) * NBUCKET) / span)], 1)] = v;
    }
    __syncthreads();
    for (int bk = w; bk < NBUCKET; bk += 16) {
      const int32_t lo = s_off[bk], sz = s_off[bk + 1] - lo;
      if (sz == 0) continue;
      if (sz <= 64) {
        const int32_t v = lane < sz ? B[lo + lane] : 0x7FFFFFFF;
        int32_t pos = 0;
        for (int j = 0; j < sz; ++j) pos += __builtin_amdgcn_readlane(v, j) < v ? 1 : 0;
        if (lane < sz) col[s + lo + pos] = v;
      } else {
        int32_t bmn = 0x7FFFFFFF, bmx = 0;
        for (int q = lane; q < sz; q += 64) {
          const int32_t v = B[lo + q];
          bmn = min(bmn, v);
          bmx = max(bmx, v);
        }
        for (int off = 32; off > 0; off >>= 1) {
          bmn = min(bmn, __shfl_xor(bmn, off, 64));
          bmx = max(bmx, __shfl_xor(bmx, off, 64));
        }
        const int64_t bspan = (int64_t)bmx - bmn + 1;
        s_sub[w][lane] = 0;
        wave_lds_sync();
        for (int q = lane; q < sz; q += 64)
          atomicAdd(&s_sub[w][(int)(((int64_t)(B[lo + q] - bmn) * 64) / bspan)], 1);
        wave_lds_sync();
        const int32_t c = s_sub[w][lane];
        int32_t incl = c;
        for (int off = 1; off < 64; off <<= 1) {
          int32_t o = __shfl_up(incl, off, 64);
          if (lane >= off) incl += o;
        }
        const int32_t sub_lo = incl - c;
        wave_lds_sync();
        s_sub[w][lane] = sub_lo;
        wave_lds_sync();
        for (int q = lane; q < sz; q += 64) {
          const int32_t v = B[lo + q];
          A[lo + atomicAdd(&s_sub[w][(int)(((int64_t)(v - bmn) * 64) / bspan)], 1)] = v;
        }
        wave_lds_sync();
        for (int sb = 0; sb < 64; ++sb) {
          const int32_t slo = __builtin_amdgcn_readlane(sub_lo, sb), ssz = __builtin_amdgcn_readlane(c, sb);
          if (ssz == 0) continue;
          if (ssz <= 64) {
            const int32_t v = lane < ssz ? A[lo + slo + lane] : 0x7FFFFFFF;
            int32_t pos = 0;
            for (int j = 0; j < ssz; ++j) pos += __builtin_amdgcn_readlane(v, j) < v ? 1 : 0;
            if (lane < ssz) col[s + lo + slo + pos] = v;
          } else {
            for (int q = lane; q < ssz; q += 64) {
              const int32_t v = A[lo + slo + q];
              int32_t pos = 0;
              for (int j = 0; j < ssz; ++j) pos += A[lo + slo + j] < v ? 1 : 0;
              col[s + lo + slo + pos] = v;
            }
          }
        }
      }
    }
    __syncthreads();
  }
  if (tid == 0) {
    if (edges) atomicAdd(&edge_counters[(blockIdx.x & 31) * ec_stride], edges);
    __threadfence();
    s_last = atomicAdd(ticket, 1) == (int32_t)gridDim.x - 1 ? 1 : 0;
  }
  __syncthreads();
  if (!s_last) return;
  int32_t total = 0;
  if (tid < 64 && (tile_edges == nullptr || tid < 32))
    total = __hip_atomic_load(&edge_counters[tid * ec_stride], __ATOMIC_RELAXED, __HIP_MEMORY_SCOPE_AGENT);
  for (int32_t q = tid; q < n_tile_edges; q += 1024) total += tile_edges[q];
  for (int off = 32; off > 0; off >>= 1) total += __shfl_xor(total, off, 64);
  if (tid == 0) s_uniq = 0;
  __syncthreads();
  if (lane == 0 && total) atomicAdd(&s_uniq, total);
  __syncthreads();
  if (tid == 0) meta[GIGL_META_N_EDGES] = s_uniq;
}

int32_t union_build_lg2(gigl_ctx* ctx, const uint32_t* roots, const gigl_tree* tree, int32_t group_roots,
                        gigl_union* out, bool multiset_rows) {
  const int b = tree->b;
  const int f0 = tree->fanouts[0], f1 = tree->fanouts[1];
  const int64_t S0 = (int64_t)b * f0, S1 = S0 * f1, T_in = b + S0;
  hipStream_t st = ctx->stream;
  int64_t n_groups = 1;
  Lg2Args g{};
  g.roots = roots;
  g.nbr0 = tree->nbr[0];
  g.nbr1 = tree->nbr[1];
  g.cnt1 = tree->cnt[1];
  g.b = b;
  g.f0 = f0;
  g.f1 = f1;
  g.S0 = S0;
  g.whole_rows = multiset_rows ? 0 : 1;
  if (group_roots != b) {
    n_groups = b / group_roots;
    g.grouped = 1;
    g.group_roots = (uint32_t)group_roots;
    g.gdiv0 = (uint32_t)group_roots * (uint32_t)f0;
  }
  const int64_t inner = (int64_t)(b / n_groups) * (1 + f0);
  uint64_t cap = 1024;
  while (cap < (uint64_t)inner * 2) cap <<= 1;
  const int64_t n_slots = (int64_t)cap * n_groups;
  GIGL_REQUIRE(ctx, n_slots < (int64_t)1 << 31 && b + S0 + S1 < (int64_t)1 << 31, "batch too large");
  const int32_t n_tiles = (int32_t)((T_in + TILE - 1) / TILE);
  const int64_t zero_words = 256;
  int64_t need = 0;
  auto add = [&](int64_t bytes) { need += gigl_align_up(bytes, 256); };
  add(n_slots * (int64_t)sizeof(Slot));
  add(zero_words * 4);
  add(T_in * 4);
  add((int64_t)(n_tiles + 1) * 2 * 4);
  add(T_in * 4);
  add(T_in * 4);
  add(T_in * 4);
  int32_t rc = gigl_arena_reset(ctx, need + 4096);
  if (rc != GIGL_OK) return rc;
  UnionArgs a{};
  a.slots = (Slot*)gigl_arena_alloc(ctx, n_slots * (int64_t)sizeof(Slot));
  int32_t* zeros = (int32_t*)gigl_arena_alloc(ctx, zero_words * 4);
  g.slot_of = (int32_t*)gigl_arena_alloc(ctx, T_in * 4);
  int32_t* tile_counts = (int32_t*)gigl_arena_alloc(ctx, (int64_t)(n_tiles + 1) * 2 * 4);
  int32_t* big_rows = (int32_t*)gigl_arena_alloc(ctx, T_in * 4);
  int32_t* sort_rows = (int32_t*)gigl_arena_alloc(ctx, T_in * 4);
  int32_t* tiny_rows = (int32_t*)gigl_arena_alloc(ctx, T_in * 4);
  if (!a.slots || !zeros || !g.slot_of || !tile_counts || !big_rows || !sort_rows || !tiny_rows)
    return gigl_fail(ctx, GIGL_E_OOM, "arena exhausted");
  a.mask = (uint32_t)(cap - 1);
  a.overflow = out->meta + GIGL_META_OVERFLOW;
  g.alias_base = -1;
  if (tree->nbr[1] == (const uint32_t*)(out->col + out->cap_edges) && out->cap_edges + S1 < ((int64_t)1 << 31))
    g.alias_base = (int32_t)out->cap_edges;
  int32_t* cursor = zeros;
  int32_t* ticket_count = zeros + 1;
  int32_t* ticket_big = zeros + 2;
  int32_t* big_count = zeros + 3;
  int32_t* sort_count = zeros + 4;
  int32_t* tiny_count = zeros + 5;
  int32_t* edge_counters = zeros + 64;
  const int TB = 256;
  auto grid = [&](int64_t n) { return dim3((unsigned)((n + TB - 1) / TB)); };
  {
    gigl_prof_scope ps(ctx, GIGL_K_UNION_INSERT);
    hipLaunchKernelGGL(lg2_init_kernel, dim3(512), dim3(256), 0, st, (uint4*)a.slots, n_slots, zeros, zero_words,
                       out->meta);
    hipLaunchKernelGGL(lg2_insert_kernel, grid(T_in), dim3(TB), 0, st, a, g);
    hipLaunchKernelGGL(lg2_extras_kernel, grid(S0), dim3(TB), 0, st, a, g);
  }
  {
    gigl_prof_scope ps(ctx, GIGL_K_UNION_NODES);
    hipLaunchKernelGGL(lg2_count_kernel, dim3((unsigned)n_tiles), dim3(256), 0, st, a, g, tile_counts, n_tiles,
                       ticket_count);
    hipLaunchKernelGGL(lg2_assign_kernel, dim3((unsigned)n_tiles), dim3(256), 0, st, a, g, tile_counts, n_tiles,
                       out->nodes, out->meta, out->rowptr, out->rowend, cursor, edge_counters + 32, sort_rows,
                       sort_count, tiny_rows, tiny_count);
  }
  {
    gigl_prof_scope ps(ctx, GIGL_K_UNION_EDGE_SORT);
    hipLaunchKernelGGL(lg2_fill_kernel, grid(T_in), dim3(TB), 0, st, a, g, out->rowend, out->col, out->root_local,
                       out->rowptr);
  }
  {
    gigl_prof_scope ps(ctx, GIGL_K_UNION_CSR);
    {
      int64_t tb = (T_in / 16 + 255) / 256;
      if (tb > 1024) tb = 1024;
      if (tb < 16) tb = 16;
      hipLaunchKernelGGL(lg2_row_sort_tiny_kernel, dim3((unsigned)tb), dim3(256), 0, st, tiny_rows, tiny_count,
                         out->rowptr, out->rowend, out->col, edge_counters);
    }
    int64_t blocks = (T_in / 8 + 3) / 4;
    if (blocks > 256 * 16) blocks = 256 * 16;
    if (blocks < 64) blocks = 64;
    hipLaunchKernelGGL(lg2_row_sort_kernel, dim3((unsigned)blocks), dim3(256), 0, st, sort_rows, sort_count,
                       out->rowptr, out->rowend, out->col, big_rows, big_count, edge_counters);
    if (lg_big_cap_wide()) {
      GIGL_HIP_CHECK(ctx, lds_opt_in(ctx->device, 0, (const void*)lg2_row_sort_big_kernel<BIG_ROW_CAP>, 2 * BIG_ROW_CAP * (int)sizeof(int32_t)));
      hipLaunchKernelGGL(lg2_row_sort_big_kernel<BIG_ROW_CAP>, dim3(8), dim3(1024), 2 * BIG_ROW_CAP * sizeof(int32_t), st,
                       out->rowptr, out->rowend, out->col, big_rows, big_count, out->meta + GIGL_META_OVERFLOW,
                       edge_counters, ticket_big, out->meta);
    } else
    hipLaunchKernelGGL(lg2_row_sort_big_kernel<LG_BIG_CAP>, dim3(8), dim3(1024), 2 * LG_BIG_CAP * sizeof(int32_t), st,
                       out->rowptr, out->rowend, out->col, big_rows, big_count, out->meta + GIGL_META_OVERFLOW,
                       edge_counters, ticket_big, out->meta);
  }
  GIGL_HIP_CHECK(ctx, hipGetLastError());
  return GIGL_OK;
}


constexpr int LG3_CODE_BITS = 20;
constexpr uint32_t LG3_CODE_MASK = (1u << LG3_CODE_BITS) - 1u;
constexpr uint32_t LG3_EMPTY = 0xFFFFFFFFu;
constexpr int32_t LG3_XTAG = 1 << 30;
constexpr int LG3_MAX_PARTS = 16;
constexpr int LG3_NT_DEFAULT = 512;
constexpr int LG3_CAP_DEFAULT = 16384;

struct Lg3Args {
  const uint32_t* roots;
  const uint32_t* nbr0;
  const uint32_t* nbr1;
  const int32_t* cnt0;
  const int32_t* cnt1;
  int32_t b, f0, f1;
  int64_t S0;
  int32_t gr;
  int32_t S0g;
  int32_t Tg;
  int32_t n_groups;
  int32_t P;
  uint32_t cmask;
  uint32_t rmask;
  int32_t rs_shift;
  int32_t bl_shift;
  int32_t* fpw;
  int32_t* fpx;
  int32_t* lid_in;
  int32_t* rowcnt;
  int32_t alias_base;
  int32_t whole_rows;
  int32_t* overflow;
};

__device__ __forceinline__ uint32_t lg3_part(uint32_t h32, int P) { return (uint32_t)(((uint64_t)h32 * (uint32_t)P) >> 32); }

__device__ __forceinline__ int64_t lg3_gpos(const Lg3Args& a, int32_t grp, uint32_t code) {
  return code < (uint32_t)a.gr ? (int64_t)grp * a.gr + code : (int64_t)a.b + (int64_t)grp * a.S0g + (code - a.gr);
}

__device__ __forceinline__ void lg3_locate(const Lg3Args& a, int64_t t, int32_t& grp, uint32_t& code) {
  if (t < a.b) {
    grp = a.n_groups == 1 ? 0 : (int32_t)((uint32_t)t / (uint32_t)a.gr);
    code = (uint32_t)(t - (int64_t)grp * a.gr);
  } else {
    const uint32_t p = (uint32_t)(t - a.b);
    grp = a.n_groups == 1 ? 0 : (int32_t)(p / (uint32_t)a.S0g);
    code = (uint32_t)a.gr + (p - (uint32_t)grp * (uint32_t)a.S0g);
  }
}

__device__ __forceinline__ bool lg3_insert(unsigned long long* table, const Lg3Args& a, uint32_t id, uint32_t h32,
                                           uint32_t code) {
  const unsigned long long mine1 = ((unsigned long long)id << 32) | ((unsigned long long)code << 1) | 1ull;
  uint32_t s = h32 & a.cmask;
  for (uint32_t probes = 0; probes <= a.cmask; ++probes) {
    unsigned long long w = table[s];
    if (w == ~0ull) {
      w = atomicCAS(&table[s], ~0ull, mine1);
      if (w == ~0ull) return true;
    }
    if ((uint32_t)(w >> 32) == id) {
      atomicMin(&table[s], mine1 & ~1ull);
      atomicAnd(&table[s], ~1ull);
      return true;
    }
    s = (s + 1) & a.cmask;
  }
  return false;
}

__device__ __forceinline__ uint32_t lg3_lookup(const unsigned long long* table, const Lg3Args& a, uint32_t id,
                                               uint32_t h32) {
  uint32_t s = h32 & a.cmask;
  for (uint32_t probes = 0; probes <= a.cmask; ++probes) {
    const unsigned long long w = table[s];
    if (w == ~0ull) return LG3_EMPTY;
// ... 491 lines not shown
        rowend[id] = pn;
      }
    }
  }
  {
    for (int off = 32; off > 0; off >>= 1) alias_c += __shfl_xor(alias_c, off, 64);
    if (lane == 0) s_alias[w] = alias_c;
    __syncthreads();
    if (tid == 0) tile_edges[blockIdx.x] = s_alias[0] + s_alias[1] + s_alias[2] + s_alias[3];
  }
  if (blockIdx.x == 0 && tid == 0) {
    meta[GIGL_META_LEVEL0] = total0;
    meta[GIGL_META_LEVEL0 + 1] = total0 + total1;
    meta[GIGL_META_LEVEL0 + 2] = total0 + total1;
    meta[GIGL_META_N_NODES] = total0 + total1;
    rowptr[total0 + total1] = 0;
    rowend[total0 + total1] = 0;
  }
}

__global__ __launch_bounds__(256) void lg3_fill_kernel(Lg3Args a, int32_t* rowend, int32_t* col, int32_t* root_local,
                                                       const int32_t* rowptr) {
  const int64_t t = (int64_t)blockIdx.x * blockDim.x + threadIdx.x;
  const int lane = threadIdx.x & 63;
  const bool in = t < a.b + a.S0;
  const int32_t w = in ? a.fpw[t] : -1;
  const bool valid = w != -1;
  int32_t grp = 0;
  uint32_t mycode = 0;
  if (in) lg3_locate(a, t, grp, mycode);
  const uint32_t code = (uint32_t)w & 0x7FFFFFFFu;
  const bool multi = valid && w < 0;
  const int32_t lid = valid ? a.lid_in[lg3_gpos(a, grp, code)] : -1;
  if (in && t < a.b) root_local[t] = lid;
  const bool edge = in && t >= a.b && valid;
  bool e_ok = false;
  int32_t dl = 0;
  if (edge) {
    const int64_t rt = (int64_t)((uint32_t)(t - a.b) / (uint32_t)a.f0);
    const int32_t wr = a.fpw[rt];
    if (wr != -1) {
      e_ok = true;
      const int64_t rpos = (int64_t)grp * a.gr + ((uint32_t)wr & 0x7FFFFFFFu);
      dl = a.lid_in[rpos];
      if (wr >= 0 && a.rowcnt[rpos] >= 2) {
        col[rowptr[dl] + (int32_t)((uint32_t)(t - a.b) % (uint32_t)a.f0)] = lid;
        e_ok = false;
      }
    }
  }
  int total, rank, first;
  seg_rank(e_ok ? (uint32_t)dl : (0x80000000u | (uint32_t)lane), e_ok, lane, total, rank, first);
  int32_t basep = 0;
  if (e_ok && rank == 0) basep = atomicAdd(&rowend[dl], total);
  basep = __shfl(basep, first, 64);
  if (e_ok) col[basep + rank] = lid;
  if (edge && (multi || a.alias_base < 0)) {
    const int64_t p = t - a.b;
    const int c = a.cnt1[p];
    if (c > 0 && !lg3_row_is_segment(a, code, c) && lg3_contributes(a, code, mycode, c)) {
      const int32_t at = atomicAdd(&rowend[lid], c);
      const bool local = code < (uint32_t)a.gr;
      const int64_t xg = (int64_t)grp * a.S0g * a.f1;
      for (int j = 0; j < c; ++j) {
        int32_t v = (int32_t)a.nbr1[p * a.f1 + j];
        if (local) {
          int32_t x = a.fpx[p * a.f1 + j];
          v = 0;
          if (x != -1) {
            if (!(x & LG3_XTAG)) {
              const uint32_t c2 = (uint32_t)x & 0x7FFFFFFFu;
              x = c2 < (uint32_t)a.Tg ? a.lid_in[lg3_gpos(a, grp, c2)] | LG3_XTAG : a.fpx[xg + (c2 - a.Tg)];
            }
            v = x & (LG3_XTAG - 1);
          }
        }
        col[at + j] = v;
      }
    }
  }
}

int32_t union_build_lg3(gigl_ctx* ctx, const uint32_t* roots, const gigl_tree* tree, int32_t group_roots,
                        gigl_union* out, bool multiset_rows, bool* taken) {
  *taken = false;
  const int b = tree->b;
  const int f0 = tree->fanouts[0], f1 = tree->fanouts[1];
  const int64_t S0 = (int64_t)b * f0, S1 = S0 * f1, T_in = b + S0;
  const int64_t n_groups = b / group_roots;
  const int64_t gr = group_roots, Tg = gr * (1 + f0), S1g = gr * f0 * f1;
  static const int lg3_nt_env = [] {
    const char* e = getenv("GIGL_LG3_NT");
    const int v = e ? atoi(e) : 0;
    return v == 512 || v == 1024 ? v : 0;
  }();
  int lg3_nt = lg3_nt_env ? lg3_nt_env : (gr * f0 <= 64 * (int64_t)LG3_NT_DEFAULT ? LG3_NT_DEFAULT : 1024);
  if (Tg + S1g >= (int64_t)LG3_CODE_MASK || f1 > 64 || b + S0 + S1 >= ((int64_t)1 << 31) || gr * f0 > 64 * (int64_t)lg3_nt) return GIGL_OK;
  static const int64_t cap_max = [] {
    const char* e = getenv("GIGL_LG3_CAP");
    const int64_t v = e ? atoll(e) : 0;
    return v >= 1024 && v <= 16384 && (v & (v - 1)) == 0 ? v : (int64_t)LG3_CAP_DEFAULT;
  }();
  int64_t cap = 1024;
  while (cap < 2 * Tg && cap < cap_max) cap <<= 1;
  const int64_t P = (2 * Tg + cap - 1) / cap;
  if (P > LG3_MAX_PARTS) return GIGL_OK;
  if (!lg3_nt_env && n_groups * P < 256) lg3_nt = 1024;
  static const int64_t min_wgs = getenv("GIGL_LG3_MIN_WGS") ? atoll(getenv("GIGL_LG3_MIN_WGS")) : 32;
  if (n_groups * P < min_wgs) return GIGL_OK;
  int64_t rs = 64;
  int rs_log2 = 6;
  while (rs < 2 * gr) {
    rs <<= 1;
    ++rs_log2;
  }
  const int64_t n_tcnt = LG3_TC * ((gr >> 10) + 2 + ((gr * f0) >> 10) + 2);
  const size_t lds_bytes = (size_t)cap * 8 + (size_t)(rs + rs / 4 + n_tcnt) * 4;
  if (lds_bytes > 150 * 1024) return GIGL_OK;
  *taken = true;
  hipStream_t st = ctx->stream;
  const int32_t n_tiles = (int32_t)((T_in + TILE - 1) / TILE);
  constexpr int EC_STRIDE = 32;
  const int64_t zero_words = 64 + 32 * EC_STRIDE + (int64_t)(n_tiles + 1) * LG3_TC;
  int64_t need = 0;
  auto add = [&](int64_t bytes) { need += gigl_align_up(bytes, 256); };
  add(zero_words * 4);
  add((int64_t)n_tiles * 4);
  add(T_in * 4);
  add(T_in * 4);
  add(T_in * 4);
  add(S1 * 4);
  add(T_in * 4);
  add(T_in * 4);
  add(T_in * 4);
  int32_t rc = gigl_arena_reset(ctx, need + 4096);
  if (rc != GIGL_OK) return rc;
  int32_t* zeros = (int32_t*)gigl_arena_alloc(ctx, zero_words * 4);
  int32_t* tile_edges = (int32_t*)gigl_arena_alloc(ctx, (int64_t)n_tiles * 4);
  Lg3Args a{};
  a.fpw = (int32_t*)gigl_arena_alloc(ctx, T_in * 4);
  a.lid_in = (int32_t*)gigl_arena_alloc(ctx, T_in * 4);
  a.rowcnt = (int32_t*)gigl_arena_alloc(ctx, T_in * 4);
  a.fpx = (int32_t*)gigl_arena_alloc(ctx, S1 * 4);
  int32_t* big_rows = (int32_t*)gigl_arena_alloc(ctx, T_in * 4);
  int32_t* sort_rows = (int32_t*)gigl_arena_alloc(ctx, T_in * 4);
  int32_t* tiny_rows = (int32_t*)gigl_arena_alloc(ctx, T_in * 4);
  if (!zeros || !tile_edges || !a.fpw || !a.lid_in || !a.rowcnt || !a.fpx || !big_rows || !sort_rows || !tiny_rows)
    return gigl_fail(ctx, GIGL_E_OOM, "arena exhausted");
  a.roots = roots;
  a.nbr0 = tree->nbr[0];
  a.nbr1 = tree->nbr[1];
  a.cnt0 = tree->cnt[0];
  a.cnt1 = tree->cnt[1];
  a.b = b;
  a.f0 = f0;
  a.f1 = f1;
  a.S0 = S0;
  a.gr = (int32_t)gr;
  a.S0g = (int32_t)(gr * f0);
  a.Tg = (int32_t)Tg;
  a.n_groups = (int32_t)n_groups;
  a.P = (int32_t)P;
  a.cmask = (uint32_t)(cap - 1);
  a.rmask = (uint32_t)(rs - 1);
  a.rs_shift = 32 - rs_log2;
  a.bl_shift = 32 - (rs_log2 + 3);
  a.whole_rows = multiset_rows ? 0 : 1;
  a.overflow = out->meta + GIGL_META_OVERFLOW;
  a.alias_base = -1;
  if (tree->nbr[1] == (const uint32_t*)(out->col + out->cap_edges) && out->cap_edges + S1 < ((int64_t)1 << 31))
    a.alias_base = (int32_t)out->cap_edges;
  int32_t* ticket_count = zeros + 1;
  int32_t* ticket_big = zeros + 2;
  int32_t* big_count = zeros + 3;
  int32_t* sort_count = zeros + 4;
  int32_t* tiny_count = zeros + 5;
  int32_t* edge_counters = zeros + 64;
  int32_t* tile_counts = zeros + 64 + 32 * EC_STRIDE;
  const int TB = 256;
  auto grid = [&](int64_t n) { return dim3((unsigned)((n + TB - 1) / TB)); };
  GIGL_HIP_CHECK(ctx, lds_opt_in(ctx->device, 1, (const void*)lg3_dedup_kernel<1024>, 150 * 1024));
  GIGL_HIP_CHECK(ctx, lds_opt_in(ctx->device, 3, (const void*)lg3_dedup_kernel<512>, 150 * 1024));
  {
    gigl_prof_scope ps(ctx, GIGL_K_UNION_INSERT);
    hipLaunchKernelGGL(lg3_init_kernel, dim3(256), dim3(256), 0, st, a.rowcnt, T_in, zeros, zero_words, out->meta);
    if (lg3_nt == 512)
      hipLaunchKernelGGL(lg3_dedup_kernel<512>, dim3((unsigned)(n_groups * P)), dim3(512), lds_bytes, st, a, tile_counts,
                         n_tiles, ticket_count, sort_count, tiny_count);
    else
      hipLaunchKernelGGL(lg3_dedup_kernel<1024>, dim3((unsigned)(n_groups * P)), dim3(1024), lds_bytes, st, a, tile_counts,
                         n_tiles, ticket_count, sort_count, tiny_count);
  }
  {
    gigl_prof_scope ps(ctx, GIGL_K_UNION_NODES);
    hipLaunchKernelGGL(lg3_assign_kernel, dim3((unsigned)n_tiles), dim3(256), 0, st, a, tile_counts, n_tiles, out->nodes,
                       out->meta, out->rowptr, out->rowend, tile_edges, sort_rows, tiny_rows);
  }
  {
    gigl_prof_scope ps(ctx, GIGL_K_UNION_EDGE_SORT);
    hipLaunchKernelGGL(lg3_fill_kernel, grid(T_in), dim3(TB), 0, st, a, out->rowend, out->col, out->root_local, out->rowptr);
  }
  {
    gigl_prof_scope ps(ctx, GIGL_K_UNION_CSR);
    {
      static const int64_t tiny_div = getenv("GIGL_LG3_TINY_DIV") ? atoll(getenv("GIGL_LG3_TINY_DIV")) : 4;
      int64_t tb = (T_in / (tiny_div > 0 ? tiny_div : 4) + 255) / 256;
      if (tb > 4096) tb = 4096;
      if (tb < 16) tb = 16;
      hipLaunchKernelGGL(lg2_row_sort_tiny_kernel, dim3((unsigned)tb), dim3(256), 0, st, tiny_rows, tiny_count,
                         out->rowptr, out->rowend, out->col, edge_counters, EC_STRIDE);
    }
    int64_t blocks = (T_in / 8 + 3) / 4;
    if (blocks > 256 * 16) blocks = 256 * 16;
    if (blocks < 64) blocks = 64;
    hipLaunchKernelGGL(lg2_row_sort_kernel, dim3((unsigned)blocks), dim3(256), 0, st, sort_rows, sort_count, out->rowptr,
                       out->rowend, out->col, big_rows, big_count, edge_counters, EC_STRIDE);
    if (lg_big_cap_wide()) {
      GIGL_HIP_CHECK(ctx, lds_opt_in(ctx->device, 4, (const void*)lg2_row_sort_big_kernel<BIG_ROW_CAP>, 2 * BIG_ROW_CAP * (int)sizeof(int32_t)));
      hipLaunchKernelGGL(lg2_row_sort_big_kernel<BIG_ROW_CAP>, dim3(8), dim3(1024), 2 * BIG_ROW_CAP * sizeof(int32_t), st, out->rowptr,
                       out->rowend, out->col, big_rows, big_count, out->meta + GIGL_META_OVERFLOW, edge_counters,
                       ticket_big, out->meta, EC_STRIDE, (const int32_t*)tile_edges, n_tiles);
    } else
    hipLaunchKernelGGL(lg2_row_sort_big_kernel<LG_BIG_CAP>, dim3(8), dim3(1024), 2 * LG_BIG_CAP * sizeof(int32_t), st, out->rowptr,
                       out->rowend, out->col, big_rows, big_count, out->meta + GIGL_META_OVERFLOW, edge_counters,
                       ticket_big, out->meta, EC_STRIDE, (const int32_t*)tile_edges, n_tiles);
  }
  GIGL_HIP_CHECK(ctx, hipGetLastError());
  return GIGL_OK;
}

}

extern "C" {

int32_t gigl_union_capacity(int32_t b, const int32_t* fanouts, int32_t hops, int64_t* cap_nodes,
                            int64_t* cap_edges) {
  if (!fanouts || hops < 1 || hops > GIGL_MAX_HOPS || b < 0) return GIGL_E_INVALID_ARG;
  int64_t parents = b, edges = 0;
  for (int k = 0; k < hops; ++k) {
    parents *= fanouts[k];
    edges += parents;
  }
  if (cap_nodes) *cap_nodes = edges + b;
  if (cap_edges) *cap_edges = edges;
  return GIGL_OK;
}

int32_t gigl_union_build(gigl_ctx* ctx, const uint32_t* roots, const gigl_tree* tree,
                         gigl_union* out) {
  if (!ctx) return GIGL_E_INVALID_ARG;
  GIGL_REQUIRE(ctx, tree, "null argument");
  return gigl_union_build_groups(ctx, roots, tree, tree->b, out);
}

int32_t gigl_union_build_groups(gigl_ctx* ctx, const uint32_t* roots, const gigl_tree* tree,
                                int32_t group_roots, gigl_union* out) {
  return gigl_union_build_impl(ctx, roots, tree, group_roots, out, 0);
}

}

int32_t gigl_union_build_impl(gigl_ctx* ctx, const uint32_t* roots, const gigl_tree* tree, int32_t group_roots,
                              gigl_union* out, int32_t leaf_global) {
  if (!ctx) return GIGL_E_INVALID_ARG;
  GIGL_REQUIRE(ctx, tree && out && (roots || tree->b == 0), "null argument");
  GIGL_REQUIRE(ctx, !leaf_global || tree->hops <= 2, "leaf-global union needs hops <= 2");
  GIGL_REQUIRE(ctx, out->meta && out->nodes && out->rowptr && out->rowend && out->col && out->root_local,
               "union output buffers are null");
  const int hops = tree->hops, b = tree->b;
  GIGL_REQUIRE(ctx, hops >= 1 && hops <= GIGL_MAX_HOPS && b >= 0, "bad tree");
  int64_t cap_nodes, cap_edges;
  gigl_union_capacity(b, tree->fanouts, hops, &cap_nodes, &cap_edges);
  GIGL_REQUIRE(ctx, out->cap_nodes >= cap_nodes && out->cap_edges >= cap_edges,
               "union buffers too small: need %lld nodes / %lld edges", (long long)cap_nodes,
               (long long)cap_edges);
  GIGL_HIP_CHECK(ctx, hipSetDevice(ctx->device));
  hipStream_t st = ctx->stream;
  if (b == 0) {
    GIGL_HIP_CHECK(ctx, hipMemsetAsync(out->meta, 0, GIGL_META_LEN * sizeof(int32_t), st));
    GIGL_HIP_CHECK(ctx, hipMemsetAsync(out->rowptr, 0, sizeof(int32_t), st));
    GIGL_HIP_CHECK(ctx, hipMemsetAsync(out->rowend, 0, sizeof(int32_t), st));
    return GIGL_OK;
  }
  if (leaf_global && hops == 2 && !getenv("GIGL_UNION_GENERIC")) {
    GIGL_REQUIRE(ctx, group_roots >= 1 && b % group_roots == 0, "group_roots=%d does not divide b=%d", group_roots, b);
    static const bool keep_lg2 = getenv("GIGL_UNION_LG2") != nullptr;
    if (!keep_lg2) {
      bool taken = false;
      const int32_t rc3 = union_build_lg3(ctx, roots, tree, group_roots, out, (leaf_global & 2) != 0, &taken);
      if (rc3 != GIGL_OK || taken) return rc3;
    }
    return union_build_lg2(ctx, roots, tree, group_roots, out, (leaf_global & 2) != 0);
  }

  UnionArgs a{};
  a.roots = roots;
  a.b = b;
  a.hops = hops;
  a.leaf_global = leaf_global ? 1 : 0;
  int64_t T = b, parents = b;
  for (int k = 0; k < hops; ++k) {
    a.nbr[k] = tree->nbr[k];
    a.fan[k] = tree->fanouts[k];
    a.off[k] = T;
    parents *= tree->fanouts[k];
    T += parents;
  }
  a.off[hops] = T;
  a.T = T;
  GIGL_REQUIRE(ctx, T < (int64_t)1 << 31, "batch too large: %lld stream positions", (long long)T);
  int64_t n_groups = 1;
  if (group_roots != b) {
    GIGL_REQUIRE(ctx, group_roots >= 1 && b % group_roots == 0, "group_roots=%d does not divide b=%d", group_roots, b);
    n_groups = b / group_roots;
    a.grouped = 1;
    a.group_roots = (uint32_t)group_roots;
    int64_t per_group = group_roots;
    for (int k = 0; k < hops; ++k) {
      per_group *= tree->fanouts[k];
      a.gdiv[k] = (uint32_t)per_group;
    }
  }
  const int64_t E = T - b;
  const int64_t max_rows = a.off[hops - 1];
  uint64_t cap = 1024, ecap = 1024;
  int64_t inner = b / n_groups, width = b / n_groups;
  for (int k = 0; k + 1 < hops; ++k) {
    width *= tree->fanouts[k];
    inner += width;
  }
  const uint64_t want = a.leaf_global ? (uint64_t)inner * 4 : (uint64_t)(T / n_groups) * 3;
  while (cap * 2 < want) cap <<= 1;
  while (ecap * 2 < (uint64_t)(E / n_groups) * 3) ecap <<= 1;
  a.mask = (uint32_t)(cap - 1);
  const int64_t n_slots = (int64_t)cap * n_groups, n_ekeys = (int64_t)ecap * n_groups;
  GIGL_REQUIRE(ctx, n_slots < (int64_t)1 << 31, "batch too large: %lld table slots", (long long)n_slots);
  const int32_t n_tiles = (int32_t)((T + TILE - 1) / TILE);

  int64_t need = 0;
  auto add = [&](int64_t bytes) { need += gigl_align_up(bytes, 256); };
  const int64_t zero_words = cap_nodes + 1 + 64;
  add(n_ekeys * 8);
  add(n_slots * (int64_t)sizeof(Slot));
  add(zero_words * 4);
  add(T * 4);
  add((int64_t)(n_tiles + 1) * MAXL * 4);
  add(cap_nodes * 4);
  add(E + 256);
  add((E + 1) * 8);
  int32_t rc = gigl_arena_reset(ctx, need + 4096);
  if (rc != GIGL_OK) return rc;
  unsigned long long* ekeys = (unsigned long long*)gigl_arena_alloc(ctx, n_ekeys * 8);
  a.slots = (Slot*)gigl_arena_alloc(ctx, n_slots * (int64_t)sizeof(Slot));
  int32_t* zeros = (int32_t*)gigl_arena_alloc(ctx, zero_words * 4);
  a.slot_of = (int32_t*)gigl_arena_alloc(ctx, T * 4);
  int32_t* tile_counts = (int32_t*)gigl_arena_alloc(ctx, (int64_t)(n_tiles + 1) * MAXL * 4);
  int32_t* big_rows = (int32_t*)gigl_arena_alloc(ctx, cap_nodes * 4);
  uint8_t* winner = (uint8_t*)gigl_arena_alloc(ctx, E + 256);
  int2* pairs = (int2*)gigl_arena_alloc(ctx, (E + 1) * 8);
  if (!ekeys || !a.slots || !zeros || !big_rows || !winner || !a.slot_of || !pairs || !tile_counts)
    return gigl_fail(ctx, GIGL_E_OOM, "arena exhausted");
  a.root_parent = winner;
  a.alias_base = -1;
  a.cnt_last = tree->cnt[hops - 1];
  if (a.leaf_global && hops == 2 && tree->nbr[1] == (const uint32_t*)(out->col + out->cap_edges) &&
      out->cap_edges + (a.off[2] - a.off[1]) < ((int64_t)1 << 31))
    a.alias_base = (int32_t)out->cap_edges;
  a.overflow = out->meta + GIGL_META_OVERFLOW;
  int32_t* rowcnt = zeros;
  int32_t* big_count = zeros + cap_nodes + 1;

  const int TB = 256;
  auto grid = [&](int64_t n) { return dim3((unsigned)((n + TB - 1) / TB)); };
  {
    gigl_prof_scope ps(ctx, GIGL_K_UNION_INSERT);
// ... 42 lines not shown
```

Measured before the change: 10.91 billion.

## Fuse fused2 prepare kernels, fold guard into union sort, pre-zero work counters

Merges the fused2 scale and image kernels, plus the hs scale update, into one prepare kernel. Each block recomputes the abs-max reductions redundantly, which removes the cross-block atomic handoff and the separate launches. The prepare step moves earlier, into the gather stage. The level-guard check moves into the last union row-sort kernel, so the separate guard kernel launch is skipped. Work-list counters now live in per-hop slots in the ctx and are zeroed by the previous stage's plan kernel instead of extra zero kernels, which cuts launches at the cost of added slot bookkeeping and redundant per-block reductions.

After: 10.98 billion, median of 2. Within noise of the previous version (+0.6%).

```diff
diff --git a/gigl_amd/csrc/agg.hip b/gigl_amd/csrc/agg.hip
--- a/gigl_amd/csrc/agg.hip
+++ b/gigl_amd/csrc/agg.hip
@@ -1196,82 +1196,89 @@
   }
 }
 
-__global__ __launch_bounds__(256) void fused2_images_kernel(const float* __restrict__ hs, const float* __restrict__ f2,
-                                                            const float* __restrict__ w1, int K, const float* __restrict__ w2,
-                                                            int n_out, _Float16* __restrict__ w1img,
-                                                            _Float16* __restrict__ w2img) {
+constexpr int F2P_NT = 512;
+__device__ __forceinline__ float f2p_absmax(const float* __restrict__ x, int n, int tid) {
+  float m = 0.f;
+  const float4* x4 = reinterpret_cast<const float4*>(x);
+  const int n4 = ((reinterpret_cast<uintptr_t>(x) & 15) == 0) ? n / 4 : 0;
+#pragma unroll 8
+  for (int i = tid; i < n4; i += F2P_NT) {
+    const float4 v = x4[i];
+    const float a = fmaxf(fmaxf(fabsf(v.x), fabsf(v.y)), fmaxf(fabsf(v.z), fabsf(v.w)));
+    m = fmaxf(m, a == a ? a : 0.f);
+  }
+  for (int i = n4 * 4 + tid; i < n; i += F2P_NT) {
+    const float v = fabsf(x[i]);
+    m = fmaxf(m, v == v ? v : 0.f);
+  }
+  return m;
+}
+
+__global__ __launch_bounds__(F2P_NT) void fused2_prepare_kernel(const float* __restrict__ w1, int K, const float* __restrict__ b1,
+                                                                const float* __restrict__ w2, int n_out, float s_a,
+                                                                float* __restrict__ hs, float* __restrict__ f2,
+                                                                _Float16* __restrict__ w1img, _Float16* __restrict__ w2img) {
+  __shared__ float s_m[3][F2P_NT / 64];
+  const int tid = threadIdx.x;
+  float m1 = f2p_absmax(w1, F2_HID * K, tid);
+  float mb = b1 ? f2p_absmax(b1, F2_HID, tid) : 0.f;
+  float m2 = f2p_absmax(w2, n_out * 2 * F2_HID, tid);
+#pragma unroll
+  for (int o = 32; o >= 1; o >>= 1) {
+    m1 = fmaxf(m1, __shfl_xor(m1, o, 64));
+    mb = fmaxf(mb, __shfl_xor(mb, o, 64));
+    m2 = fmaxf(m2, __shfl_xor(m2, o, 64));
+  }
+  if ((tid & 63) == 0) {
+    s_m[0][tid >> 6] = m1;
+    s_m[1][tid >> 6] = mb;
+    s_m[2][tid >> 6] = m2;
+  }
+  __syncthreads();
+#pragma unroll
+  for (int i = 0; i < F2P_NT / 64; ++i) {
+    m1 = fmaxf(m1, s_m[0][i]);
+    mb = fmaxf(mb, s_m[1][i]);
+    m2 = fmaxf(m2, s_m[2][i]);
+  }
+  const float inf = __uint_as_float(0x7F800000u);
+  const float s_w = (m1 > 0.f && m1 < inf) ? hs_pow2_scale(m1) : 1.f;
+  float bound = (float)K * 1073741824.f * (1.f / s_a) * (1.f / s_w) + mb;
+  if (!(bound > 0.f) || !(bound < inf)) bound = 1.f;
+  const float s_h = hs_pow2_scale(bound) * 0.5f;
+  const float s_w2 = (m2 > 0.f && m2 < inf) ? hs_pow2_scale(m2) : 1.f;
+  if (blockIdx.x == 0 && tid == 0) {
+    hs[0] = s_a;
+    hs[1] = s_w;
+    hs[2] = (1.f / s_a) * (1.f / s_w);
+    f2[0] = s_h;
+    f2[1] = s_w2;
+    f2[2] = (1.f / s_h) * (1.f / s_w2);
+  }
   const int nc = (K + 31) >> 5;
   const int n1 = 2 * nc * 128 * 32, n2 = 2 * 4 * F2_N2 * 32;
-  const int i = blockIdx.x * 256 + threadIdx.x;
-  if (i < n1) {
-    const int kpos = i & 31, c = (i >> 5) & 127, blk = i >> 12;
-    const int tn = blk / nc, ch = blk - tn * nc;
-    const int k = 32 * ch + f2_perm(kpos);
-    const float x = k < K ? w1[(int64_t)(128 * tn + c) * K + k] * hs[1] : 0.f;
-    const _Float16 a1 = (_Float16)x;
-    _Float16* img = w1img + (int64_t)blk * F2_IMG1 + split_lds_off(c, kpos);
-    img[0] = a1;
-    img[F2_IMG1 / 2] = (_Float16)(x - (float)a1);
-  } else if (i < n1 + n2) {
-    const int e = i - n1;
-    const int kpos = e & 31, rest = e >> 5, n = rest % F2_N2, blk = rest / F2_N2;
-    const int k = 32 * blk + f2_perm(kpos);
-    float x = 0.f;
-    if (n < n_out) x = w2[(int64_t)n * 2 * F2_HID + k];
-    else if (n >= F2_N2 / 2 && n - F2_N2 / 2 < n_out) x = w2[(int64_t)(n - F2_N2 / 2) * 2 * F2_HID + F2_HID + k];
-    x *= f2[1];
-    const _Float16 a1 = (_Float16)x;
-    _Float16* img = w2img + (int64_t)blk * F2_IMG2 + split_lds_off(n, kpos);
-    img[0] = a1;
-    img[F2_IMG2 / 2] = (_Float16)(x - (float)a1);
-  }
-}
-
-__global__ __launch_bounds__(256) void fused2_scale_kernel(const float* __restrict__ hs, const float* __restrict__ b1,
-                                                           const float* __restrict__ w2, int n_w2, int K1,
-                                                           float* __restrict__ f2) {
-  __shared__ float s_m[2][4];
-  const int tid = threadIdx.x, gt = blockIdx.x * 256 + tid, stride = gridDim.x * 256;
-  float mb = 0.f, mw = 0.f;
-  if (b1)
-    for (int i = gt; i < F2_HID; i += stride) {
-      const float v = fabsf(b1[i]);
-      mb = fmaxf(mb, v == v ? v : 0.f);
-    }
-  for (int i = gt; i < n_w2; i += stride) {
-    const float v = fabsf(w2[i]);
-    mw = fmaxf(mw, v == v ? v : 0.f);
-  }
-#pragma unroll
-  for (int o = 32; o >= 1; o >>= 1) {
-    mb = fmaxf(mb, __shfl_xor(mb, o, 64));
-    mw = fmaxf(mw, __shfl_xor(mw, o, 64));
-  }
-  if ((tid & 63) == 0) {
-    s_m[0][tid >> 6] = mb;
-    s_m[1][tid >> 6] = mw;
-  }
-  __syncthreads();
-  if (tid == 0) {
-    for (int i = 1; i < 4; ++i) {
-      mb = fmaxf(mb, s_m[0][i]);
-      mw = fmaxf(mw, s_m[1][i]);
-    }
-    uint32_t* acc = reinterpret_cast<uint32_t*>(f2) + 4;
-    atomicMax(acc, __float_as_uint(mb));
-    atomicMax(acc + 1, __float_as_uint(mw));
-    __threadfence();
-    if (atomicAdd(acc + 2, 1u) == gridDim.x - 1) {
-      const float b = __uint_as_float(atomicExch(acc, 0u)), w = __uint_as_float(atomicExch(acc + 1, 0u));
-      acc[2] = 0u;
-      const float inf = __uint_as_float(0x7F800000u);
-      float bound = (float)K1 * 1073741824.f * (1.f / hs[0]) * (1.f / hs[1]) + b;
-      if (!(bound > 0.f) || !(bound < inf)) bound = 1.f;
-      const float s_h = hs_pow2_scale(bound) * 0.5f;
-      const float s_w2 = (w > 0.f && w < inf) ? hs_pow2_scale(w) : 1.f;
-      f2[0] = s_h;
-      f2[1] = s_w2;
-      f2[2] = (1.f / s_h) * (1.f / s_w2);
+  for (int i = blockIdx.x * F2P_NT + tid; i < n1 + n2; i += gridDim.x * F2P_NT) {
+    if (i < n1) {
+      const int kpos = i & 31, c = (i >> 5) & 127, blk = i >> 12;
+      const int tn = blk / nc, ch = blk - tn * nc;
+      const int k = 32 * ch + f2_perm(kpos);
+      const float x = k < K ? w1[(int64_t)(128 * tn + c) * K + k] * s_w : 0.f;
+      const _Float16 a1 = (_Float16)x;
+      _Float16* img = w1img + (int64_t)blk * F2_IMG1 + split_lds_off(c, kpos);
+      img[0] = a1;
+      img[F2_IMG1 / 2] = (_Float16)(x - (float)a1);
+    } else {
+      const int e = i - n1;
+      const int kpos = e & 31, rest = e >> 5, n = rest % F2_N2, blk = rest / F2_N2;
+      const int k = 32 * blk + f2_perm(kpos);
+      float x = 0.f;
+      if (n < n_out) x = w2[(int64_t)n * 2 * F2_HID + k];
+      else if (n >= F2_N2 / 2 && n - F2_N2 / 2 < n_out) x = w2[(int64_t)(n - F2_N2 / 2) * 2 * F2_HID + F2_HID + k];
+      x *= s_w2;
+      const _Float16 a1 = (_Float16)x;
+      _Float16* img = w2img + (int64_t)blk * F2_IMG2 + split_lds_off(n, kpos);
+      img[0] = a1;
+      img[F2_IMG2 / 2] = (_Float16)(x - (float)a1);
     }
   }
 }
@@ -4320,14 +4327,13 @@
 int64_t gigl_fused2_w2h_bytes(int32_t k1) { return fused2_img1_bytes(k1) + (int64_t)2 * 4 * F2_IMG2 * 2; }
 int32_t gigl_fused2_row_floats() { return F2_N2; }
 
-int32_t gigl_fused2_prepare(gigl_ctx* ctx, const float* hs_dev, const float* b1, const float* w1, const float* w2, int32_t n_out,
-                            int32_t k1, float* f2, void* w2h) {
-  hipLaunchKernelGGL(fused2_scale_kernel, dim3(24), dim3(256), 0, ctx->stream, hs_dev, b1, w2, n_out * 2 * F2_HID, k1, f2);
+int32_t gigl_fused2_prepare(gigl_ctx* ctx, float s_a, const float* b1, const float* w1, const float* w2, int32_t n_out,
+                            int32_t k1, float* hs_dev, float* f2, void* w2h) {
   _Float16* img1 = reinterpret_cast<_Float16*>(w2h);
   _Float16* img2 = reinterpret_cast<_Float16*>(reinterpret_cast<char*>(w2h) + fused2_img1_bytes(k1));
   const int n = 2 * ((k1 + 31) / 32) * 128 * 32 + 2 * 4 * F2_N2 * 32;
-  hipLaunchKernelGGL(fused2_images_kernel, dim3((unsigned)((n + 255) / 256)), dim3(256), 0, ctx->stream, hs_dev,
-                     (const float*)f2, w1, k1, w2, n_out, img1, img2);
+  hipLaunchKernelGGL(fused2_prepare_kernel, dim3((unsigned)((n + 2 * F2P_NT - 1) / (2 * F2P_NT))), dim3(F2P_NT), 0, ctx->stream, w1,
+                     k1, b1, w2, n_out, s_a, hs_dev, f2, img1, img2);
   GIGL_HIP_CHECK(ctx, hipGetLastError());
   return GIGL_OK;
 }
diff --git a/gigl_amd/csrc/common.h b/gigl_amd/csrc/common.h
--- a/gigl_amd/csrc/common.h
+++ b/gigl_amd/csrc/common.h
@@ -12,7 +12,10 @@
 
 #include "../../include/gigl_hip.h"
 
+#include "work_slots.h"
+
 #define GIGL_WAVE 64
+constexpr int64_t GIGL_WORK_SLOT_BYTES = 64 * 32 * 4;
 
 struct gigl_ctx {
   int device = 0;
@@ -31,6 +34,7 @@
   double prof_acc_ms[16] = {0};
   int64_t prof_acc_n[16] = {0};
   void* sampler_table = nullptr;
+  int32_t* work_counts = nullptr;
   uint32_t* crc_shift_tbl = nullptr;
   uint32_t* enc_tables = nullptr;
   int32_t enc_tables_d = -1;
@@ -108,7 +112,7 @@
 int32_t gigl_linear_weight_grad_parts(gigl_ctx* ctx, const float* dy, const float* a, const float* relu_y, const int32_t* m_dev,
                                       int64_t m_cap, int32_t n, int32_t k, float* part, float* partb);
 int32_t gigl_union_build_impl(gigl_ctx* ctx, const uint32_t* roots, const gigl_tree* tree, int32_t group_roots,
-                              gigl_union* out, int32_t leaf_global);
+                              gigl_union* out, int32_t leaf_global, int32_t guard_rows = 0, bool* guarded = nullptr);
 void gigl_scan_i64(gigl_ctx* ctx, const int64_t* sizes, int64_t n, int64_t cap, int64_t* out, int32_t* status);
 int32_t gigl_gather_reduce_mixed(gigl_ctx* ctx, const void* src, int32_t src_dtype, int32_t d, const uint32_t* gather_ids,
                                  const int32_t* rowptr, const int32_t* rowend, const int32_t* col,
@@ -179,8 +183,8 @@
 bool gigl_fused2_shape_ok(int32_t d0, int32_t hid, int32_t n_out);
 int64_t gigl_fused2_w2h_bytes(int32_t k1);
 int32_t gigl_fused2_row_floats();
-int32_t gigl_fused2_prepare(gigl_ctx* ctx, const float* hs_dev, const float* b1, const float* w1, const float* w2, int32_t n_out,
-                            int32_t k1, float* f2, void* w2h);
+int32_t gigl_fused2_prepare(gigl_ctx* ctx, float s_a, const float* b1, const float* w1, const float* w2, int32_t n_out,
+                            int32_t k1, float* hs_dev, float* f2, void* w2h);
 int32_t gigl_linear_fused2(gigl_ctx* ctx, const float* a_tiled, const float* bias, const int32_t* m_dev, int64_t m_cap,
                            int32_t k, float* y2, const float* self_src, const uint32_t* self_ids, int32_t d_mean,
                            int32_t self_ld, const float* hs_scale, const float* f2, const void* w2h,
diff --git a/gigl_amd/csrc/ctx.hip b/gigl_amd/csrc/ctx.hip
--- a/gigl_amd/csrc/ctx.hip
+++ b/gigl_amd/csrc/ctx.hip
@@ -115,6 +115,14 @@
     return GIGL_E_HIP;
   }
   c->own_stream = true;
+  if (hipMalloc((void**)&c->work_counts, (size_t)(GIGL_WORK_SLOTS * GIGL_WORK_SLOT_BYTES)) != hipSuccess ||
+      hipMemsetAsync(c->work_counts, 0, (size_t)(GIGL_WORK_SLOTS * GIGL_WORK_SLOT_BYTES), c->stream) != hipSuccess ||
+      hipStreamSynchronize(c->stream) != hipSuccess) {
+    if (c->work_counts) hipFree(c->work_counts);
+    hipStreamDestroy(c->stream);
+    delete c;
+    return GIGL_E_HIP;
+  }
   *out = c;
   return GIGL_OK;
 }
@@ -124,6 +132,7 @@
   hipSetDevice(ctx->device);
   if (ctx->stream) hipStreamSynchronize(ctx->stream);
   if (ctx->arena) hipFree(ctx->arena);
+  if (ctx->work_counts) hipFree(ctx->work_counts);
   gigl_sampler_table_free(ctx);
   if (ctx->crc_shift_tbl) hipFree(ctx->crc_shift_tbl);
   if (ctx->enc_tables) hipFree(ctx->enc_tables);
diff --git a/gigl_amd/csrc/pipeline.hip b/gigl_amd/csrc/pipeline.hip
--- a/gigl_amd/csrc/pipeline.hip
+++ b/gigl_amd/csrc/pipeline.hip
@@ -235,12 +235,15 @@
   if (s == 0)
     return gigl_sample_khop(ctx, p->graph, roots, p->b, p->fanouts, p->hops, sampling_seed, mode, &p->tree);
   if (s == 1) {
+    const int32_t guard_rows = (int32_t)(p->act_rows < 0x7FFFFFFF ? p->act_rows : 0x7FFFFFFF);
+    bool guarded = false;
     int32_t rc = gigl_union_build_impl(ctx, roots, &p->tree, p->group_roots, &p->un,
-                                       p->leaf_global ? (1 | (p->graph->multi ? 2 : 0)) : 0);
+                                       p->leaf_global ? (1 | (p->graph->multi ? 2 : 0)) : 0, guard_rows, &guarded);
     if (rc != GIGL_OK) return rc;
-    hipLaunchKernelGGL(guard_levels_kernel, dim3(1), dim3(64), 0, ctx->stream, p->un.meta, p->hops,
-                       (int32_t)(p->act_rows < 0x7FFFFFFF ? p->act_rows : 0x7FFFFFFF));
-    GIGL_HIP_CHECK(ctx, hipGetLastError());
+    if (!guarded) {
+      hipLaunchKernelGGL(guard_levels_kernel, dim3(1), dim3(64), 0, ctx->stream, p->un.meta, p->hops, guard_rows);
+      GIGL_HIP_CHECK(ctx, hipGetLastError());
+    }
     if (p->efeat) {
       const int64_t rows_cap = gigl_level_rows(p->wide, p->b, p->fanouts, L, L - 1);
       int64_t blocks = (rows_cap + 3) / 4;
@@ -325,6 +328,11 @@
   const bool two_src = p->tiled && p->two_source && (l > 0 || p->feat->dtype == GIGL_DTYPE_F32 || self_half);
   const int32_t nkc = p->tiled ? ((two_src ? d : 2 * d) + 31) / 32 : 0;
   if (((s - 2) & 1) == 0) {
+    if (l == 0 && fused2_on(p)) {
+      const int32_t rc = gigl_fused2_prepare(ctx, p->hs_sa, p->bias[0], p->w[0], p->w[1], p->dims[2], 2 * d, p->hs_dev,
+                                             p->f2_dev, p->w2h);
+      if (rc != GIGL_OK) return rc;
+    }
     if (p->tiled) {
       if (l == 0)
         return gigl_gather_reduce_mixed(
@@ -348,8 +356,10 @@
   const int act = (l < L - 1 || p->act_last) ? 1 : 0;
   const float* hs_scale = nullptr;
   if (l == 0 && p->hs0 && p->tiled) {
-    const int32_t rc = gigl_hs_scale_update(ctx, p->w[0], (int64_t)p->dims[1] * 2 * d, p->hs_sa, p->hs_dev);
-    if (rc != GIGL_OK) return rc;
+    if (!fused2_on(p)) {
+      const int32_t rc = gigl_hs_scale_update(ctx, p->w[0], (int64_t)p->dims[1] * 2 * d, p->hs_sa, p->hs_dev);
+      if (rc != GIGL_OK) return rc;
+    }
     hs_scale = p->hs_dev;
   }
   if (l >= 1 && two_src && p->hs0 && !p->proj && p->hs_layer[l] && hs_layers_on()) {
@@ -363,13 +373,10 @@
     return gigl_linear_tiled(ctx, p->abuf, p->w[l], p->bias[l], n_rows, rows_cap, 2 * d, p->dims[l + 1], act,
                              p->hbuf[l & 1], p->hbuf[(l - 1) & 1], nullptr, d, d, p->hs_layer[l]);
   }
-  if (l == 0 && fused2_on(p)) {
-    int32_t rc = gigl_fused2_prepare(ctx, p->hs_dev, p->bias[0], p->w[0], p->w[1], p->dims[2], 2 * d, p->f2_dev, p->w2h);
-    if (rc != GIGL_OK) return rc;
+  if (l == 0 && fused2_on(p))
     return gigl_linear_fused2(ctx, p->abuf, p->bias[0], n_rows, rows_cap, 2 * d, p->hbuf[0], (const float*)p->feat->rows,
                               p->un.nodes, d, d, hs_scale, p->f2_dev, p->w2h,
                               getenv("GIGL_F2_ALL_WR") ? nullptr : p->un.meta + GIGL_META_LEVEL0);
-  }
   if (two_src)
     return gigl_linear_tiled(ctx, p->abuf, p->w[l], p->bias[l], n_rows, rows_cap, 2 * d, p->dims[l + 1], act,
                              p->hbuf[l & 1], l == 0 ? (const float*)p->feat->rows : p->hbuf[(l - 1) & 1],
diff --git a/gigl_amd/csrc/sample.hip b/gigl_amd/csrc/sample.hip
--- a/gigl_amd/csrc/sample.hip
+++ b/gigl_amd/csrc/sample.hip
@@ -440,6 +440,7 @@
 struct WorkLists {
   uint32_t* items;
   int32_t* count;
+  int32_t* zero_next;
   int64_t cap;
   int32_t iters;
   int32_t wgs;
@@ -454,6 +455,7 @@
 }
 
 __global__ void work_counts_zero_kernel(int32_t* count) { count[threadIdx.x * WORK_CNT_STRIDE] = 0; }
+static_assert(WORK_LISTS * WORK_CNT_STRIDE * 4 == GIGL_WORK_SLOT_BYTES, "a slot holds one hop's counters");
 
 __global__ __launch_bounds__(256) void plan_rows_kernel(ExpandArgs a, RangeTable tb, RowDesc* __restrict__ desc,
                                                         int64_t* heavy_list, int32_t* heavy_count, WorkLists wl) {
@@ -461,6 +463,7 @@
   __shared__ int32_t s_base;
   const uint32_t p = blockIdx.x * 256u + threadIdx.x;
   const int lane = threadIdx.x & 63, w = threadIdx.x >> 6;
+  if (blockIdx.x == 0 && threadIdx.x < WORK_LISTS && wl.zero_next) wl.zero_next[threadIdx.x * WORK_CNT_STRIDE] = 0;
   bool real = false;
   if (p <= (uint32_t)a.n_parents) {
     RowDesc d{};
@@ -1136,10 +1139,17 @@
   return GIGL_OK;
 }
 
+int32_t* work_slot(gigl_ctx* ctx, int slot) {
+  return slot < 0 ? nullptr : reinterpret_cast<int32_t*>(reinterpret_cast<char*>(ctx->work_counts) + (int64_t)slot * GIGL_WORK_SLOT_BYTES);
+}
+
 int32_t run_expand(gigl_ctx* ctx, const ExpandArgs& a_in, const RangeTable& tb, bool covered,
-                   int64_t* heavy_list, int32_t* heavy_count, RowDesc* desc) {
+                   int64_t* heavy_list, int32_t* heavy_count, RowDesc* desc, const gigl_work_slot_rule& slots) {
   ExpandArgs a = a_in;
+  GIGL_REQUIRE(ctx, ctx->work_counts, "the ctx has no work-list counters");
   if (a.f > GIGL_FAST_FANOUT) {
+    if (slots.zero_next >= 0)
+      hipLaunchKernelGGL(work_counts_zero_kernel, dim3(1), dim3(WORK_LISTS), 0, ctx->stream, work_slot(ctx, slots.zero_next));
     gigl_prof_scope ps(ctx, GIGL_K_EXPAND);
     int64_t wgs = a.n_parents < 8192 ? a.n_parents : 8192;
     hipLaunchKernelGGL(expand_wide_kernel, dim3((unsigned)wgs), dim3(256), 0, ctx->stream, a);
@@ -1160,9 +1170,9 @@
   WorkLists wl{};
   wl.cap = work_list_cap(a.n_parents);
   wl.items = reinterpret_cast<uint32_t*>(desc + a.n_parents + 1);
-  wl.count = reinterpret_cast<int32_t*>(wl.items + (int64_t)WORK_LISTS * wl.cap);
-  wl.count = reinterpret_cast<int32_t*>(((uintptr_t)wl.count + 127) & ~(uintptr_t)127);
-  hipLaunchKernelGGL(work_counts_zero_kernel, dim3(1), dim3(WORK_LISTS), 0, ctx->stream, wl.count);
+  wl.count = work_slot(ctx, slots.use);
+  wl.zero_next = work_slot(ctx, slots.zero_next);
+  if (slots.zero_first) hipLaunchKernelGGL(work_counts_zero_kernel, dim3(1), dim3(WORK_LISTS), 0, ctx->stream, wl.count);
   {
     gigl_prof_scope ps(ctx, GIGL_K_EXPAND);
     hipLaunchKernelGGL(plan_rows_kernel, dim3((unsigned)(a.n_parents / 256 + 1)), dim3(256), 0, ctx->stream, a, tb,
@@ -1379,8 +1389,11 @@
         hipLaunchKernelGGL(expand_replace_kernel, dim3((unsigned)blocks), dim3(256), 0, ctx->stream, a);
       GIGL_HIP_CHECK(ctx, hipGetLastError());
     } else {
-      rc = run_expand(ctx, a, tb, covered, heavy_list, heavy_count, desc);
-      if (rc != GIGL_OK) return rc;
+      rc = run_expand(ctx, a, tb, covered, heavy_list, heavy_count, desc, gigl_work_slot(hops, k));
+      if (rc != GIGL_OK) {
+        if (k > 0) hipLaunchKernelGGL(work_counts_zero_kernel, dim3(1), dim3(WORK_LISTS), 0, ctx->stream, work_slot(ctx, 0));
+        return rc;
+      }
     }
     a.anc[k] = out->nbr[k];
     parents *= fanouts[k];
@@ -1437,8 +1450,11 @@
     a.hash_add = (int32_t)((uint32_t)sampling_seed * (uint32_t)(k + 1));
     a.out_nbr = out->nbr[k];
     a.out_cnt = out->cnt[k];
-    rc = run_expand(ctx, a, tb, true, nullptr, nullptr, desc);
-    if (rc != GIGL_OK) return rc;
+    rc = run_expand(ctx, a, tb, true, nullptr, nullptr, desc, gigl_work_slot(hops, k));
+    if (rc != GIGL_OK) {
+      if (k > 0) hipLaunchKernelGGL(work_counts_zero_kernel, dim3(1), dim3(WORK_LISTS), 0, ctx->stream, work_slot(ctx, 0));
+      return rc;
+    }
     a.anc[k] = out->nbr[k];
     parents *= fanouts[k];
   }
@@ -1487,7 +1503,7 @@
   a.ex_nodes = nodes;
   a.ex_ksum = ksums;
   a.row_div = (uint32_t)world;
-  return run_expand(ctx, a, tb, covered, heavy_list, heavy_count, desc);
+  return run_expand(ctx, a, tb, covered, heavy_list, heavy_count, desc, gigl_work_slot(1, 0));
 }
 
 int32_t gigl_sample_positives(gigl_ctx* ctx, gigl_graph* g_out, const uint32_t* roots, int32_t b,
@@ -1531,7 +1547,7 @@
   rc = ensure_table(ctx, bound == ~0ULL ? (1ull << 20) : (bound + 1 < cap ? bound + 1 : cap));
   if (rc != GIGL_OK) return rc;
   const RangeTable tb = ((TableOwner*)ctx->sampler_table)->t;
-  return run_expand(ctx, a, tb, bound != ~0ULL && bound < tb.dom, heavy_list, heavy_count, desc);
-}
-
-}
+  return run_expand(ctx, a, tb, bound != ~0ULL && bound < tb.dom, heavy_list, heavy_count, desc, gigl_work_slot(1, 0));
+}
+
+}
diff --git a/gigl_amd/csrc/union.hip b/gigl_amd/csrc/union.hip
--- a/gigl_amd/csrc/union.hip
+++ b/gigl_amd/csrc/union.hip
@@ -1280,8 +1280,9 @@
 __global__ __launch_bounds__(1024) void lg2_row_sort_big_kernel(const int32_t* rowptr, int32_t* rowend, int32_t* col,
                                                                 const int32_t* big_rows, const int32_t* big_count,
                                                                 int32_t* overflow, int32_t* edge_counters,
-                                                                int32_t* ticket, int32_t* meta, int ec_stride = 1,
-                                                                const int32_t* tile_edges = nullptr, int32_t n_tile_edges = 0) {
+                                                                int32_t* ticket, int32_t* meta, int ec_stride,
+                                                                const int32_t* tile_edges, int32_t n_tile_edges,
+                                                                int guard_hops, int32_t guard_rows) {
   extern __shared__ int32_t lds[];
   int32_t* A = lds;
   int32_t* B = lds + CAP;
@@ -1459,11 +1460,20 @@
   __syncthreads();
   if (lane == 0 && total) atomicAdd(&s_uniq, total);
   __syncthreads();
-  if (tid == 0) meta[GIGL_META_N_EDGES] = s_uniq;
+  if (tid == 0) {
+    meta[GIGL_META_N_EDGES] = s_uniq;
+    bool over = false;
+    for (int l = 0; l < guard_hops; ++l) over = over || meta[GIGL_META_LEVEL0 + l] > guard_rows;
+    if (over) {
+      for (int l = 0; l < guard_hops; ++l) meta[GIGL_META_LEVEL0 + l] = 0;
+      atomicAdd(&meta[GIGL_META_OVERFLOW], 1);
+    }
+  }
 }
 
 int32_t union_build_lg2(gigl_ctx* ctx, const uint32_t* roots, const gigl_tree* tree, int32_t group_roots,
-                        gigl_union* out, bool multiset_rows) {
+                        gigl_union* out, bool multiset_rows, int32_t guard_rows) {
+  const int guard_hops = guard_rows > 0 ? tree->hops : 0;
   const int b = tree->b;
   const int f0 = tree->fanouts[0], f1 = tree->fanouts[1];
   const int64_t S0 = (int64_t)b * f0, S1 = S0 * f1, T_in = b + S0;
@@ -1565,11 +1575,11 @@
       GIGL_HIP_CHECK(ctx, lds_opt_in(ctx->device, 0, (const void*)lg2_row_sort_big_kernel<BIG_ROW_CAP>, 2 * BIG_ROW_CAP * (int)sizeof(int32_t)));
       hipLaunchKernelGGL(lg2_row_sort_big_kernel<BIG_ROW_CAP>, dim3(8), dim3(1024), 2 * BIG_ROW_CAP * sizeof(int32_t), st,
                        out->rowptr, out->rowend, out->col, big_rows, big_count, out->meta + GIGL_META_OVERFLOW,
-                       edge_counters, ticket_big, out->meta);
+                       edge_counters, ticket_big, out->meta, 1, (const int32_t*)nullptr, 0, guard_hops, guard_rows);
     } else
     hipLaunchKernelGGL(lg2_row_sort_big_kernel<LG_BIG_CAP>, dim3(8), dim3(1024), 2 * LG_BIG_CAP * sizeof(int32_t), st,
                        out->rowptr, out->rowend, out->col, big_rows, big_count, out->meta + GIGL_META_OVERFLOW,
-                       edge_counters, ticket_big, out->meta);
+                       edge_counters, ticket_big, out->meta, 1, (const int32_t*)nullptr, 0, guard_hops, guard_rows);
   }
   GIGL_HIP_CHECK(ctx, hipGetLastError());
   return GIGL_OK;
@@ -2227,8 +2237,9 @@
 }
 
 int32_t union_build_lg3(gigl_ctx* ctx, const uint32_t* roots, const gigl_tree* tree, int32_t group_roots,
-                        gigl_union* out, bool multiset_rows, bool* taken) {
+                        gigl_union* out, bool multiset_rows, bool* taken, int32_t guard_rows) {
   *taken = false;
+  const int guard_hops = guard_rows > 0 ? tree->hops : 0;
   const int b = tree->b;
   const int f0 = tree->fanouts[0], f1 = tree->fanouts[1];
   const int64_t S0 = (int64_t)b * f0, S1 = S0 * f1, T_in = b + S0;
@@ -2364,11 +2375,11 @@
       GIGL_HIP_CHECK(ctx, lds_opt_in(ctx->device, 4, (const void*)lg2_row_sort_big_kernel<BIG_ROW_CAP>, 2 * BIG_ROW_CAP * (int)sizeof(int32_t)));
       hipLaunchKernelGGL(lg2_row_sort_big_kernel<BIG_ROW_CAP>, dim3(8), dim3(1024), 2 * BIG_ROW_CAP * sizeof(int32_t), st, out->rowptr,
                        out->rowend, out->col, big_rows, big_count, out->meta + GIGL_META_OVERFLOW, edge_counters,
-                       ticket_big, out->meta, EC_STRIDE, (const int32_t*)tile_edges, n_tiles);
+                       ticket_big, out->meta, EC_STRIDE, (const int32_t*)tile_edges, n_tiles, guard_hops, guard_rows);
     } else
     hipLaunchKernelGGL(lg2_row_sort_big_kernel<LG_BIG_CAP>, dim3(8), dim3(1024), 2 * LG_BIG_CAP * sizeof(int32_t), st, out->rowptr,
                        out->rowend, out->col, big_rows, big_count, out->meta + GIGL_META_OVERFLOW, edge_counters,
-                       ticket_big, out->meta, EC_STRIDE, (const int32_t*)tile_edges, n_tiles);
+                       ticket_big, out->meta, EC_STRIDE, (const int32_t*)tile_edges, n_tiles, guard_hops, guard_rows);
   }
   GIGL_HIP_CHECK(ctx, hipGetLastError());
   return GIGL_OK;
@@ -2400,13 +2411,14 @@
 
 int32_t gigl_union_build_groups(gigl_ctx* ctx, const uint32_t* roots, const gigl_tree* tree,
                                 int32_t group_roots, gigl_union* out) {
-  return gigl_union_build_impl(ctx, roots, tree, group_roots, out, 0);
+  return gigl_union_build_impl(ctx, roots, tree, group_roots, out, 0, 0, nullptr);
 }
 
 }
 
 int32_t gigl_union_build_impl(gigl_ctx* ctx, const uint32_t* roots, const gigl_tree* tree, int32_t group_roots,
-                              gigl_union* out, int32_t leaf_global) {
+                              gigl_union* out, int32_t leaf_global, int32_t guard_rows, bool* guarded) {
+  if (guarded) *guarded = false;
   if (!ctx) return GIGL_E_INVALID_ARG;
   GIGL_REQUIRE(ctx, tree && out && (roots || tree->b == 0), "null argument");
   GIGL_REQUIRE(ctx, !leaf_global || tree->hops <= 2, "leaf-global union needs hops <= 2");
@@ -2432,10 +2444,13 @@
     static const bool keep_lg2 = getenv("GIGL_UNION_LG2") != nullptr;
     if (!keep_lg2) {
       bool taken = false;
-      const int32_t rc3 = union_build_lg3(ctx, roots, tree, group_roots, out, (leaf_global & 2) != 0, &taken);
+      const int32_t rc3 = union_build_lg3(ctx, roots, tree, group_roots, out, (leaf_global & 2) != 0, &taken,
+                                          guarded ? guard_rows : 0);
+      if (rc3 == GIGL_OK && taken && guarded) *guarded = guard_rows > 0;
       if (rc3 != GIGL_OK || taken) return rc3;
     }
-    return union_build_lg2(ctx, roots, tree, group_roots, out, (leaf_global & 2) != 0);
+    if (guarded) *guarded = guard_rows > 0;
+    return union_build_lg2(ctx, roots, tree, group_roots, out, (leaf_global & 2) != 0, guarded ? guard_rows : 0);
   }
 
   UnionArgs a{};
diff --git a/gigl_amd/csrc/work_slots.h b/gigl_amd/csrc/work_slots.h
--- /dev/null
+++ b/gigl_amd/csrc/work_slots.h
@@ -0,0 +1,14 @@
+#pragma once
+
+constexpr int GIGL_WORK_SLOTS = 5;
+
+struct gigl_work_slot_rule {
+  int use;
+  int zero_next;
+  int zero_first;
+};
+
+inline gigl_work_slot_rule gigl_work_slot(int hops, int k) {
+  if (hops < 2) return {GIGL_WORK_SLOTS - 1, -1, 1};
+  return {k, k + 1 < hops ? k + 1 : 0, 0};
+}
```
